# marwie/mageslam

Measured on AMD Instinct MI355X. Metric: frames/sec ORB extract+match @720p; local-BA iters/sec (50 KF, 5k pts), higher is better.
Workload: dtype u8

## Files before the change

### mageslam_amd/csrc/localmap.hip

```cpp
#include <hip/hip_runtime.h>

#include <algorithm>
#include <climits>
#include <cstring>

#include "band_index.hpp"
#include "common.hpp"
#include "lds_sort.hpp"
#include "ordered_take.hpp"

namespace mage {
namespace {

constexpr int LM_MAXT = 4096;
constexpr int LM_CAP = 8;
constexpr int LM_GROUP = 16;
static_assert(LM_MAXT <= OT_MAX_TARGETS, "keypoint indices must fit resolve_in_order's packings");

struct LmRec {
    int n;
    int lo, hi;
    int pad;
    uint32_t e[LM_CAP];
};

__global__ __launch_bounds__(SORT_THREADS) void lm_keys_kernel(LocalMapArgs a, unsigned long long* __restrict__ gkeys)
{
    __shared__ unsigned long long keys[LM_MAXT];
    const int n = (int)*a.nt, tid = threadIdx.x;
    if (*a.nq == 0) return;
    if (n > LM_MAXT) {
        if (tid == 0) atomicOr(a.status, 1u);
        return;
    }
    int P = 1;
    while (P < n) P <<= 1;
    for (int i = tid; i < max(P, SORT_THREADS); i += SORT_THREADS)
        keys[i] = i < n ? ~band_key(a.tkp[i].octave, a.tkp[i].y, (unsigned)i) : 0ull;
    __syncthreads();
    sort_desc(keys, P);
    for (int i = tid; i < n; i += SORT_THREADS) gkeys[i] = ~keys[i];
}

template <typename F>
__device__ __forceinline__ void scan_band(const LocalMapArgs& a, const unsigned long long* keys, int q, int lo, int hi,
                                          int first, int step, F visit)
{
    const float r = a.radius, px = a.qpos[2 * q], py = a.qpos[2 * q + 1];
    const float x0 = px - r, x1 = px + r, y0 = py - r, y1 = py + r;
    const int hide = a.qhide ? a.qhide[q] : -1;
    const uint8_t* qd = a.qdesc + 32ll * q;
    for (int i = lo + first; i < hi; i += step) {
        const int t = (int)(keys[i] & 0xFFFFFFu);
        const float tx = a.tkp[t].x, ty = a.tkp[t].y;
        if (!(tx >= x0 && tx <= x1 && ty >= y0 && ty <= y1) || t == hide) continue;
        const uint32_t d = hamming256(qd, a.tdesc + 32ll * t);
        if ((int)d <= a.max_dist) visit(t, (int)d);
    }
}

__global__ __launch_bounds__(1024) void lm_cand_kernel(LocalMapArgs a, const unsigned long long* __restrict__ keys,
                                                       LmRec* __restrict__ recs)
{
    const int nq = (int)*a.nq, nt = (int)*a.nt;
    if (nt > LM_MAXT || nq > (int)a.q_cap) return;
    const int q = (int)((blockIdx.x * 1024 + threadIdx.x) / LM_GROUP), sub = threadIdx.x % LM_GROUP;
    const bool live = q < nq;
    int lo = 0, hi = 0;
    if (live) {
        const float py = a.qpos[2 * q + 1], r = a.radius;
        const int oq = a.qoct[q];
        lo = lower_bound_keys(keys, nt, band_key(oq, py - r, 0u));
        hi = lower_bound_keys(keys, nt, band_key(oq, py + r, 0xFFFFFFu) + 1ull);
    }
    int n = 0;
    for (int i0 = lo; __any(live && i0 < hi); i0 += LM_GROUP) {
        bool f = false;
        uint32_t ent = 0;
        if (live && i0 + sub < hi) {
            const int i = i0 + sub;
            const int t = (int)(keys[i] & 0xFFFFFFu);
            if (mask_bit(a.mask_words, t))
                scan_band(a, keys, q, i, i + 1, 0, 1, [&](int tt, int d) {
                    f = true;
                    ent = kept_entry(tt, d);
                });
        }
        const int pos = group_append<LM_GROUP>(f, sub, n);
        if (f && pos < LM_CAP) recs[q].e[pos] = ent;
    }
    if (live && sub == 0) {
        recs[q].n = n;
        recs[q].lo = lo;
        recs[q].hi = hi;
    }
}

__global__ __launch_bounds__(1024) void lm_resolve_kernel(LocalMapArgs a, const unsigned long long* __restrict__ keys,
                                                          const LmRec* __restrict__ recs)
{
    __shared__ uint32_t m[LM_MAXT / 32];
    __shared__ int taker[LM_MAXT];
    __shared__ int list[1024];
    __shared__ uint32_t ent[64][LM_CAP];
    __shared__ uint32_t wsum[16];
    const int tid = threadIdx.x, lane = tid & 63, wave = tid >> 6;
    const int nq = (int)*a.nq, nt = (int)*a.nt;
    if (nt > LM_MAXT || nq > (int)a.q_cap) {
        if (tid == 0) atomicOr(a.status, 2u);
        return;
    }
    for (int i = tid; i < LM_MAXT / 32; i += 1024) m[i] = i < (nt + 31) / 32 ? a.mask_words[i] : 0u;
    for (int i = tid; i < LM_MAXT; i += 1024) taker[i] = OT_NO_TAKER;
    __syncthreads();
    for (int b0 = 0; b0 < nq; b0 += 1024) {
        const int q = b0 + tid;
        const bool has = q < nq && recs[q].n > 0;
        if (q < nq) a.result[q] = -1;
        const uint64_t bal = __ballot(has);
        if (lane == 0) wsum[wave] = (uint32_t)__popcll(bal);
        __syncthreads();
        int off = 0, cnt = 0;
        for (int w = 0; w < 16; w++) {
            off += w < wave ? (int)wsum[w] : 0;
            cnt += (int)wsum[w];
        }
        if (has) list[off + __popcll(bal & ((1ull << lane) - 1ull))] = q;
        __syncthreads();
        if (tid < 64)
            resolve_in_order(
                cnt, a.max_dist, a.min_diff, m, taker,
                [&](int k, bool act) {
                    const int qq = act ? list[k] : 0;
                    int n = 0, lo = 0, hi = 0;
                    if (act) {
                        n = recs[qq].n;
                        lo = recs[qq].lo;
                        hi = recs[qq].hi;
                        for (int e = 0; e < LM_CAP && e < n; e++) ent[tid][e] = recs[qq].e[e];
                    }
                    return [=, &a](auto fn) {
                        if (!act) return;
                        if (n <= LM_CAP) {
                            for (int e = 0; e < n; e++) {
                                const uint32_t v = ent[tid][e];
                                if (mask_bit(m, kept_target(v))) fn(kept_target(v), kept_dist(v));
                            }
                        } else {
                            scan_band(a, keys, qq, lo, hi, 0, 1, [&](int t, int d) {
                                if (mask_bit(m, t)) fn(t, d);
                            });
                        }
                    };
                },
                [&](int k, bool ok, int t) {
                    if (ok) a.result[list[k]] = t;
                });
        __syncthreads();
    }
    for (int i = tid; i < (nt + 31) / 32; i += 1024) a.mask_words[i] = m[i];
}

}

size_t local_map_scratch_bytes(uint32_t q_cap)
{
    return ((size_t)LM_MAXT * 8 + 255) / 256 * 256 + (size_t)std::max(q_cap, 1u) * sizeof(LmRec);
}

mage_status local_map_match_launch(const LocalMapArgs& a, void* scratch, hipStream_t st)
{
    unsigned long long* keys = static_cast<unsigned long long*>(scratch);
    LmRec* recs = reinterpret_cast<LmRec*>(static_cast<char*>(scratch) + ((size_t)LM_MAXT * 8 + 255) / 256 * 256);
    if (a.keys)
        keys = const_cast<unsigned long long*>(a.keys);
    else
        launch("localmap.keys", lm_keys_kernel, dim3(1), dim3(SORT_THREADS), 0, st, a, keys);
    const unsigned groups = (unsigned)(((size_t)std::max(a.q_cap, 1u) * LM_GROUP + 1023) / 1024);
    launch("localmap.cand", lm_cand_kernel, dim3(groups), dim3(1024), 0, st, a, (const unsigned long long*)keys, recs);
    launch("localmap.resolve", lm_resolve_kernel, dim3(1), dim3(1024), 0, st, a, (const unsigned long long*)keys,
           (const LmRec*)recs);
    MAGE_HIP(hipGetLastError());
    return MAGE_OK;
}

}

extern "C" mage_status mage_local_map_match(const float* query_pos, const int32_t* query_octave, const uint8_t* query_desc,
                                            const int32_t* query_hide, uint32_t n_query, const mage_keypoint* target_kp,
                                            const uint8_t* target_desc, uint32_t n_target, uint8_t* mask, float radius,
                                            int32_t max_distance, int32_t min_difference, int32_t* result, int device)
{
    using namespace mage;
    MAGE_REQUIRE(mask && (n_target == 0 || (target_kp && target_desc)) &&
                     (n_query == 0 || (query_pos && query_octave && query_desc && result)),
                 MAGE_EINVAL, "null argument");
    MAGE_REQUIRE(n_target <= (uint32_t)LM_MAXT, MAGE_EUNSUPPORTED, "more than 4096 target keypoints");
    MAGE_REQUIRE(max_distance >= -1 && max_distance <= 256, MAGE_EINVAL, "maxHammingDist must be in [-1, 256]");
    if (n_query == 0) return MAGE_OK;
    mage_status r = bind_device(device);
    if (r != MAGE_OK) return r;
    HostScratch* sp = host_scratch(device, SCRATCH_LOCALMAP);
    if (!sp) return MAGE_EDEVICE;
    HostScratch& S = *sp;
    auto al = [](size_t v) { return (v + 255) & ~(size_t)255; };
    const size_t oqp = 0, oqo = al(oqp + 8ull * n_query), oqh = al(oqo + 4ull * n_query), oqd = al(oqh + 4ull * n_query),
                 otk = al(oqd + 32ull * n_query), otd = al(otk + 28ull * std::max(n_target, 1u)),
                 ocnt = al(otd + 32ull * std::max(n_target, 1u)), omw = al(ocnt + 8), ores = al(omw + 4 * (LM_MAXT / 32)),
                 ost = al(ores + 4ull * n_query), oscr = al(ost + 4), total = oscr + local_map_scratch_bytes(n_query);
    if ((r = S.buf.reserve(total)) != MAGE_OK || (r = S.host.reserve(oscr)) != MAGE_OK) return r;
    char* b = S.buf.as<char>();
    char* h = S.host.as<char>();
    std::memcpy(h + oqp, query_pos, 8ull * n_query);
    std::memcpy(h + oqo, query_octave, 4ull * n_query);
    if (query_hide) std::memcpy(h + oqh, query_hide, 4ull * n_query);
    else std::memset(h + oqh, 0xFF, 4ull * n_query);
    std::memcpy(h + oqd, query_desc, 32ull * n_query);
    if (n_target) {
        std::memcpy(h + otk, target_kp, 28ull * n_target);
        std::memcpy(h + otd, target_desc, 32ull * n_target);
    }
    const uint32_t counts[2] = {n_query, n_target};
    std::memcpy(h + ocnt, counts, 8);
    uint32_t* mw = reinterpret_cast<uint32_t*>(h + omw);
    std::memset(mw, 0, 4 * (LM_MAXT / 32));
    for (uint32_t t = 0; t < n_target; t++)
        if (mask[t]) mw[t >> 5] |= 1u << (t & 31);
    std::memset(h + ost, 0, 4);
    MAGE_HIP(hipMemcpyAsync(b, h, oscr, hipMemcpyHostToDevice, S.st));
    LocalMapArgs a{};
    a.qpos = reinterpret_cast<const float*>(b + oqp);
    a.qoct = reinterpret_cast<const int*>(b + oqo);
    a.qhide = reinterpret_cast<const int*>(b + oqh);
    a.qdesc = reinterpret_cast<const uint8_t*>(b + oqd);
    a.nq = reinterpret_cast<const uint32_t*>(b + ocnt);
    a.q_cap = n_query;
    a.tkp = reinterpret_cast<const mage_keypoint*>(b + otk);
    a.tdesc = reinterpret_cast<const uint8_t*>(b + otd);
    a.nt = reinterpret_cast<const uint32_t*>(b + ocnt) + 1;
    a.mask_words = reinterpret_cast<uint32_t*>(b + omw);
    a.radius = radius;
    a.max_dist = max_distance;
    a.min_diff = min_difference;
    a.result = reinterpret_cast<int*>(b + ores);
    a.status = reinterpret_cast<uint32_t*>(b + ost);
    if ((r = local_map_match_launch(a, b + oscr, S.st)) != MAGE_OK) return r;
    MAGE_HIP(hipMemcpyAsync(h + omw, b + omw, oscr - omw, hipMemcpyDeviceToHost, S.st));
    MAGE_HIP(hipStreamSynchronize(S.st));
    MAGE_REQUIRE(*reinterpret_cast<const uint32_t*>(h + ost) == 0, MAGE_EDEVICE, "local map match: bad counts");
    std::memcpy(result, h + ores, 4ull * n_query);
    for (uint32_t t = 0; t < n_target; t++) mask[t] = (mw[t >> 5] >> (t & 31)) & 1u;
    return MAGE_OK;
}
```

### mageslam_amd/csrc/radius.hip

```cpp
#include <hip/hip_runtime.h>

#include <algorithm>
#include <climits>
#include <cstring>

#include "common.hpp"
#include "band_index.hpp"
#include "lds_sort.hpp"

namespace mage {
namespace {

constexpr int RM_MAXT = 4096;
constexpr int RM_STAGE = 2048;

struct RadiusParams {
    const mage_keypoint* qkp;
    const float* qpos;
    const uint8_t* qmask;
    const uint8_t* qdesc;
    const uint32_t* nq;
    long long q_pitch;
    const mage_keypoint* tkp;
    const uint8_t* tmask;
    const uint8_t* tdesc;
    const uint32_t* nt;
    long long t_pitch;
    float radius;
    int max_dist, min_diff;
    unsigned cap;
    int* res;
    mage_dmatch* out;
    uint32_t* n_out;
    uint32_t* status;
    const unsigned long long* bkeys;
    const float2* bxy;
    const uint4* bdesc;
    RadiusFollow follow;
};

__device__ __forceinline__ void radius_done(const RadiusParams& p, int pr, uint32_t n)
{
    p.n_out[pr] = n;
    const RadiusFollow& g = p.follow;
    if (!g.exec) return;
    const uint32_t ns = *g.ns;
    const bool weak = radius_pass_weak(n, ns, g.min_matches, g.ratio);
    const uint32_t run = g.exec[g.k] && weak;
    g.exec[g.k + 1] = run;
    *g.nq_next = run ? ns : 0u;
}

constexpr int RM_GROUP = 16;
constexpr int RM_GROUPS = SORT_THREADS / RM_GROUP;

__device__ __forceinline__ unsigned group_min(unsigned v)
{
#pragma unroll
    for (int off = RM_GROUP / 2; off > 0; off >>= 1) v = min(v, (unsigned)__shfl_xor((int)v, off));
    return v;
}

__device__ void radius_post(const RadiusParams& p, int pr, const int* res, int nq, int ntr, int* bestD, int* cnt,
                            int* wsum, int& s_base)
{
    const int tid = threadIdx.x, lane = tid & 63;
    const int wave = __builtin_amdgcn_readfirstlane(tid >> 6);
    for (int i = tid; i < ntr; i += SORT_THREADS) {
        bestD[i] = INT_MAX;
        cnt[i] = 0;
    }
    __syncthreads();
    for (int q = tid; q < nq; q += SORT_THREADS) {
        const int v = res[q];
        if (v >= 0) atomicMin(&bestD[v >> 9], v & 0x1FF);
    }
    __syncthreads();
    for (int q = tid; q < nq; q += SORT_THREADS) {
        const int v = res[q];
        if (v >= 0 && (v & 0x1FF) == bestD[v >> 9]) atomicAdd(&cnt[v >> 9], 1);
    }
    if (tid == 0) s_base = 0;
    __syncthreads();
    for (int q0 = 0; q0 < nq; q0 += SORT_THREADS) {
        const int q = q0 + tid;
        const int v = q < nq ? res[q] : -1;
        const bool keep = v >= 0 && (v & 0x1FF) == bestD[v >> 9] && cnt[v >> 9] == 1;
        const unsigned long long b = __ballot(keep);
        const int before = __popcll(b & ((1ull << lane) - 1ull));
        if (lane == 0) wsum[wave] = __popcll(b);
        __syncthreads();
        int off = s_base;
        for (int w = 0; w < wave; w++) off += wsum[w];
        if (keep) {
            const int pos = off + before;
            if (pos < (int)p.cap) {
                mage_dmatch m;
                m.query_idx = q;
                m.train_idx = v >> 9;
                m.img_idx = 0;
                m.distance = (float)(v & 0x1FF);
                p.out[(long long)pr * p.cap + pos] = m;
            }
        }
        __syncthreads();
        if (tid == 0) {
            int tot = 0;
            for (int w = 0; w < SORT_THREADS / kWave; w++) tot += wsum[w];
            s_base += tot;
        }
        __syncthreads();
    }
    if (tid == 0) radius_done(p, pr, (uint32_t)s_base);
}

template <bool FUSED>
__global__ __launch_bounds__(SORT_THREADS) void radius_match_kernel(RadiusParams p)
{
    __shared__ unsigned long long keys[RM_MAXT];
    __shared__ float2 sxy[RM_STAGE];
    __shared__ uint4 sdesc[2 * RM_STAGE];
    __shared__ int wsum[SORT_THREADS / kWave];
    __shared__ int s_base;
    const int pr = blockIdx.x, tid = threadIdx.x;
    const int nq = (int)p.nq[pr], ntr = (int)p.nt[pr];
    const mage_keypoint* qkp = p.qkp + pr * p.q_pitch;
    const mage_keypoint* tkp = p.tkp + pr * p.t_pitch;
    const uint8_t* qdesc = p.qdesc + pr * p.q_pitch * 32;
    const uint8_t* tdesc = p.tdesc + pr * p.t_pitch * 32;
    const uint8_t* qmask = p.qmask ? p.qmask + pr * p.q_pitch : nullptr;
    const uint8_t* tmask = p.tmask ? p.tmask + pr * p.t_pitch : nullptr;
    const float* qpos = p.qpos ? p.qpos + 2 * pr * p.q_pitch : nullptr;
    int* res = p.res + pr * p.q_pitch;
    if (nq == 0) {
        if (FUSED && tid == 0) radius_done(p, pr, 0);
        return;
    }
    if (ntr > RM_MAXT || ntr > p.t_pitch || nq > p.q_pitch) {
        if (tid == 0 && blockIdx.y == 0) {
            radius_done(p, pr, 0);
            atomicOr(p.status, ntr > RM_MAXT ? 1u : 2u);
        }
        return;
    }
    const bool staged = ntr <= RM_STAGE;
    if (p.bkeys) {
        const long long tb = pr * p.t_pitch;
        for (int i = tid; i < ntr; i += SORT_THREADS) keys[i] = p.bkeys[tb + i];
        if (staged)
            for (int i = tid; i < 2 * ntr; i += SORT_THREADS) {
                sdesc[i] = p.bdesc[2 * tb + i];
                if (!(i & 1)) sxy[i >> 1] = p.bxy[tb + (i >> 1)];
            }
        __syncthreads();
    } else {
    int P = 1;
    while (P < ntr) P <<= 1;
    for (int i = tid; i < max(P, SORT_THREADS); i += SORT_THREADS)
        keys[i] = i < ntr ? ~band_key(tkp[i].octave, tkp[i].y, (unsigned)i) : 0ull;
    __syncthreads();
    sort_desc(keys, P);
    for (int i = tid; i < ntr; i += SORT_THREADS) keys[i] = ~keys[i];
    __syncthreads();
    if (staged) {
        for (int i = tid; i < 2 * ntr; i += SORT_THREADS) {
            const int t = (int)(keys[i >> 1] & 0xFFFFFFu);
            sdesc[i] = reinterpret_cast<const uint4*>(tdesc + 32 * (long long)t)[i & 1];
            if (!(i & 1)) {
                const bool off = tmask && !tmask[t];
                sxy[i >> 1] = off ? make_float2(__int_as_float(0x7FC00000), 0.f) : make_float2(tkp[t].x, tkp[t].y);
            }
        }
        __syncthreads();
    }
    }

    const float r = p.radius;
    const int group = tid / RM_GROUP, sub = tid % RM_GROUP;
    for (int q = (int)blockIdx.y * RM_GROUPS + group; q < nq; q += RM_GROUPS * (int)gridDim.y) {
        if (qmask && !qmask[q]) {
            if (sub == 0) res[q] = -1;
            continue;
        }
        const float px = qpos ? qpos[2 * q] : qkp[q].x, py = qpos ? qpos[2 * q + 1] : qkp[q].y;
        const int oq = qkp[q].octave;
        const float x0 = px - r, x1 = px + r, y0 = py - r, y1 = py + r;
        const int lo = lower_bound_keys(keys, ntr, band_key(oq, y0, 0u));
        const int hi = lower_bound_keys(keys, ntr, band_key(oq, y1, 0xFFFFFFu) + 1ull);
        uint4 qa = *reinterpret_cast<const uint4*>(qdesc + 32 * (long long)q);
        uint4 qb = *reinterpret_cast<const uint4*>(qdesc + 32 * (long long)q + 16);
        unsigned bestk = 0xFFFFFFFFu;
        for (int i = lo + sub; i < hi; i += RM_GROUP) {
            const int t = (int)(keys[i] & 0xFFFFFFu);
            uint4 ta, tb;
            if (staged) {
                const float2 xy = sxy[i];
                if (!(xy.x >= x0 && xy.x <= x1 && xy.y >= y0 && xy.y <= y1)) continue;
                ta = sdesc[2 * i];
                tb = sdesc[2 * i + 1];
            } else {
                const float tx = tkp[t].x, ty = tkp[t].y;
                if (!(tx >= x0 && tx <= x1 && ty >= y0 && ty <= y1)) continue;
                if (tmask && !tmask[t]) continue;
                ta = *reinterpret_cast<const uint4*>(tdesc + 32 * (long long)t);
                tb = *reinterpret_cast<const uint4*>(tdesc + 32 * (long long)t + 16);
            }
            const unsigned d = __popc(qa.x ^ ta.x) + __popc(qa.y ^ ta.y) + __popc(qa.z ^ ta.z) + __popc(qa.w ^ ta.w) +
                               __popc(qb.x ^ tb.x) + __popc(qb.y ^ tb.y) + __popc(qb.z ^ tb.z) + __popc(qb.w ^ tb.w);
            bestk = min(bestk, d << 12 | (unsigned)t);
        }
        bestk = group_min(bestk);
        const int best = bestk == 0xFFFFFFFFu ? INT_MAX : (int)(bestk >> 12), tbest = (int)(bestk & 0xFFFu);
        if (best > p.max_dist) {
            if (sub == 0) res[q] = -1;
            continue;
        }
        unsigned sec = (unsigned)(p.max_dist + 1);
        for (int i = lo + sub; i < hi; i += RM_GROUP) {
            const int t = (int)(keys[i] & 0xFFFFFFu);
            if (t >= tbest) continue;
            uint4 ta, tb;
            if (staged) {
                const float2 xy = sxy[i];
                if (!(xy.x >= x0 && xy.x <= x1 && xy.y >= y0 && xy.y <= y1)) continue;
                ta = sdesc[2 * i];
                tb = sdesc[2 * i + 1];
            } else {
                const float tx = tkp[t].x, ty = tkp[t].y;
                if (!(tx >= x0 && tx <= x1 && ty >= y0 && ty <= y1)) continue;
                if (tmask && !tmask[t]) continue;
                ta = *reinterpret_cast<const uint4*>(tdesc + 32 * (long long)t);
                tb = *reinterpret_cast<const uint4*>(tdesc + 32 * (long long)t + 16);
            }
            const unsigned d = __popc(qa.x ^ ta.x) + __popc(qa.y ^ ta.y) + __popc(qa.z ^ ta.z) + __popc(qa.w ^ ta.w) +
                               __popc(qb.x ^ tb.x) + __popc(qb.y ^ tb.y) + __popc(qb.z ^ tb.z) + __popc(qb.w ^ tb.w);
            sec = min(sec, d);
        }
        sec = group_min(sec);
        if (sub == 0) res[q] = ((int)sec - best > p.min_diff) ? (tbest << 9 | best) : -1;
    }
    if constexpr (FUSED) {
        __syncthreads();
        int* bestD = reinterpret_cast<int*>(keys);
        radius_post(p, pr, res, nq, ntr, bestD, bestD + RM_MAXT, wsum, s_base);
    }
}

__global__ __launch_bounds__(SORT_THREADS) void radius_post_kernel(RadiusParams p)
{
    __shared__ int bestD[RM_MAXT];
    __shared__ int cnt[RM_MAXT];
    __shared__ int wsum[SORT_THREADS / kWave];
    __shared__ int s_base;
    const int pr = blockIdx.x;
    const int nq = (int)p.nq[pr], ntr = (int)p.nt[pr];
    if (nq == 0) {
        if (threadIdx.x == 0) radius_done(p, pr, 0);
        return;
    }
    if (ntr > RM_MAXT || ntr > p.t_pitch || nq > p.q_pitch) return;
    radius_post(p, pr, p.res + pr * p.q_pitch, nq, ntr, bestD, cnt, wsum, s_base);
}

__global__ __launch_bounds__(SORT_THREADS) void radius_band_index_kernel(const mage_keypoint* __restrict__ tkp,
                                                                         const uint8_t* __restrict__ tdesc,
                                                                         const uint32_t* __restrict__ nt, long long t_pitch,
                                                                         unsigned long long* __restrict__ bkeys,
                                                                         float2* __restrict__ bxy, uint4* __restrict__ bdesc)
{
    __shared__ unsigned long long keys[RM_MAXT];
    const int set = blockIdx.x, tid = threadIdx.x;
    const int ntr = (int)nt[set];
    if (ntr > RM_MAXT || ntr > t_pitch) return;
    const long long tb = set * t_pitch;
    const mage_keypoint* k = tkp + tb;
    int P = 1;
    while (P < ntr) P <<= 1;
    for (int i = tid; i < max(P, SORT_THREADS); i += SORT_THREADS)
        keys[i] = i < ntr ? ~band_key(k[i].octave, k[i].y, (unsigned)i) : 0ull;
    __syncthreads();
    sort_desc(keys, P);
    for (int i = tid; i < ntr; i += SORT_THREADS) {
        const unsigned long long key = ~keys[i];
        const int t = (int)(key & 0xFFFFFFu);
        bkeys[tb + i] = key;
        bxy[tb + i] = make_float2(k[t].x, k[t].y);
        const uint4* d = reinterpret_cast<const uint4*>(tdesc + 32 * (tb + t));
        bdesc[2 * (tb + i)] = d[0];
        bdesc[2 * (tb + i) + 1] = d[1];
    }
}

}

mage_status radius_band_index_launch(const mage_keypoint* d_target_kp, const uint8_t* d_target_desc,
                                     const uint32_t* d_n_target, int64_t target_pitch, uint32_t sets,
                                     unsigned long long* d_keys, float* d_xy, uint32_t* d_desc, hipStream_t st)
{
    if (sets == 0) return MAGE_OK;
    launch("match.radius_index", radius_band_index_kernel, dim3(sets), dim3(SORT_THREADS), 0, st, d_target_kp,
           d_target_desc, d_n_target, (long long)target_pitch, d_keys, reinterpret_cast<float2*>(d_xy),
           reinterpret_cast<uint4*>(d_desc));
    MAGE_HIP(hipGetLastError());
    return MAGE_OK;
}

mage_status radius_match_launch(const RadiusParams& p, uint32_t pairs, hipStream_t st)
{
    const uint32_t split = pairs >= 128 ? 1u : std::min(64u, (256u + pairs - 1) / pairs);
    if (split == 1) {
        launch("match.radius", radius_match_kernel<true>, dim3(pairs), dim3(SORT_THREADS), 0, st, p);
    } else {
        launch("match.radius", radius_match_kernel<false>, dim3(pairs, split), dim3(SORT_THREADS), 0, st, p);
        MAGE_HIP(hipGetLastError());
        launch("match.radius_post", radius_post_kernel, dim3(pairs), dim3(SORT_THREADS), 0, st, p);
    }
    MAGE_HIP(hipGetLastError());
    return MAGE_OK;
}

}

extern "C" {

mage_status mage_radius_match(const mage_keypoint* query_kp, const float* query_pos, const uint8_t* query_mask,
                              const uint8_t* query_desc, uint32_t n_query, const mage_keypoint* target_kp,
                              const uint8_t* target_mask, const uint8_t* target_desc, uint32_t n_target,
                              float radius, int32_t max_distance, int32_t min_difference, mage_dmatch* out,
                              uint32_t cap, uint32_t* n)
{
    using namespace mage;
    MAGE_REQUIRE(n && (cap == 0 || out), MAGE_EINVAL, "null output");
    *n = 0;
    MAGE_REQUIRE((n_query == 0 || (query_kp && query_desc)) && (n_target == 0 || (target_kp && target_desc)),
                 MAGE_EINVAL, "null input");
    MAGE_REQUIRE(n_target <= (uint32_t)RM_MAXT, MAGE_EUNSUPPORTED, "more than 4096 target keypoints");
    MAGE_REQUIRE(max_distance >= -1 && max_distance <= 256, MAGE_EINVAL, "maxHammingDist must be in [-1, 256]");
    if (n_query == 0 || n_target == 0) return MAGE_OK;
    int dev = 0;
    MAGE_HIP(hipGetDevice(&dev));
    mage_status r = bind_device(dev);
    if (r != MAGE_OK) return r;
    HostScratch* sp = host_scratch(dev, SCRATCH_RADIUS);
    if (!sp) return MAGE_EDEVICE;
    HostScratch& S = *sp;
    auto al = [](size_t v) { return (v + 255) & ~(size_t)255; };
    const size_t oqk = 0, otk = al(oqk + 28ull * n_query), oqd = al(otk + 28ull * n_target),
                 otd = al(oqd + 32ull * n_query), oqp = al(otd + 32ull * n_target), oqm = al(oqp + 8ull * n_query),
                 otm = al(oqm + n_query), ocnt = al(otm + n_target), ores = al(ocnt + 16),
                 oout = al(ores + 4ull * n_query), total = oout + 16ull * n_query;
    if ((r = S.buf.reserve(total)) != MAGE_OK || (r = S.host.reserve(total)) != MAGE_OK) return r;
    char* b = S.buf.as<char>();
    char* h = S.host.as<char>();
    std::memcpy(h + oqk, query_kp, 28ull * n_query);
    std::memcpy(h + otk, target_kp, 28ull * n_target);
    std::memcpy(h + oqd, query_desc, 32ull * n_query);
    std::memcpy(h + otd, target_desc, 32ull * n_target);
    if (query_pos) std::memcpy(h + oqp, query_pos, 8ull * n_query);
    if (query_mask) std::memcpy(h + oqm, query_mask, n_query);
    if (target_mask) std::memcpy(h + otm, target_mask, n_target);
    const uint32_t counts[4] = {n_query, n_target, 0, 0};
    std::memcpy(h + ocnt, counts, 16);
    MAGE_HIP(hipMemcpyAsync(b, h, ores, hipMemcpyHostToDevice, S.st));
    RadiusParams p{};
    p.qkp = reinterpret_cast<const mage_keypoint*>(b + oqk);
    p.qpos = query_pos ? reinterpret_cast<const float*>(b + oqp) : nullptr;
    p.qmask = query_mask ? reinterpret_cast<const uint8_t*>(b + oqm) : nullptr;
    p.qdesc = reinterpret_cast<const uint8_t*>(b + oqd);
    p.nq = reinterpret_cast<const uint32_t*>(b + ocnt);
    p.q_pitch = n_query;
    p.tkp = reinterpret_cast<const mage_keypoint*>(b + otk);
    p.tmask = target_mask ? reinterpret_cast<const uint8_t*>(b + otm) : nullptr;
    p.tdesc = reinterpret_cast<const uint8_t*>(b + otd);
    p.nt = reinterpret_cast<const uint32_t*>(b + ocnt) + 1;
    p.t_pitch = n_target;
    p.radius = radius;
    p.max_dist = max_distance;
    p.min_diff = min_difference;
    p.cap = n_query;
    p.res = reinterpret_cast<int*>(b + ores);
    p.out = reinterpret_cast<mage_dmatch*>(b + oout);
    p.n_out = reinterpret_cast<uint32_t*>(b + ocnt) + 2;
    p.status = reinterpret_cast<uint32_t*>(b + ocnt) + 3;
    if ((r = radius_match_launch(p, 1, S.st)) != MAGE_OK) return r;
    MAGE_HIP(hipMemcpyAsync(h + ocnt, b + ocnt, total - ocnt, hipMemcpyDeviceToHost, S.st));
    MAGE_HIP(hipStreamSynchronize(S.st));
    const uint32_t m = reinterpret_cast<const uint32_t*>(h + ocnt)[2];
    if (m > 0 && cap > 0) std::memcpy(out, h + oout, 16ull * (m < cap ? m : cap));
    *n = m < cap ? m : cap;
    MAGE_REQUIRE(m <= cap, MAGE_ECAPACITY, "output capacity too small");
    return MAGE_OK;
}

mage_status mage_radius_match_batch_device(const mage_keypoint* d_query_kp, const float* d_query_pos,
                                           const uint8_t* d_query_desc, int64_t query_pitch,
                                           const uint32_t* d_n_query, const mage_keypoint* d_target_kp,
                                           const uint8_t* d_target_desc, int64_t target_pitch,
                                           const uint32_t* d_n_target, uint32_t pairs, float radius,
                                           int32_t max_distance, int32_t min_difference, int32_t* d_scratch,
                                           mage_dmatch* d_out, uint32_t cap, uint32_t* d_n, uint32_t* d_status,
                                           mage_stream stream)
{
    using namespace mage;
    if (pairs == 0) return MAGE_OK;
    MAGE_REQUIRE(d_query_kp && d_query_desc && d_n_query && d_target_kp && d_target_desc && d_n_target &&
                     d_scratch && d_out && d_n && d_status,
                 MAGE_EINVAL, "null buffer");
    MAGE_REQUIRE(query_pitch > 0 && target_pitch > 0, MAGE_EINVAL, "pitches must be positive");
    MAGE_REQUIRE(max_distance >= -1 && max_distance <= 256, MAGE_EINVAL, "maxHammingDist must be in [-1, 256]");
    RadiusParams p{};
    p.qkp = d_query_kp;
    p.qpos = d_query_pos;
    p.qdesc = d_query_desc;
    p.nq = d_n_query;
    p.q_pitch = query_pitch;
    p.tkp = d_target_kp;
    p.tdesc = d_target_desc;
    p.nt = d_n_target;
    p.t_pitch = target_pitch;
    p.radius = radius;
    p.max_dist = max_distance;
    p.min_diff = min_difference;
    p.cap = cap;
    p.res = d_scratch;
    p.out = d_out;
    p.n_out = d_n;
    p.status = d_status;
    return radius_match_launch(p, pairs, (hipStream_t)stream);
}

}

namespace mage {
mage_status radius_match_indexed(const mage_keypoint* d_query_kp, const float* d_query_pos, const uint8_t* d_query_desc,
                                 int64_t query_pitch, const uint32_t* d_n_query, const mage_keypoint* d_target_kp,
                                 const uint8_t* d_target_desc, int64_t target_pitch, const uint32_t* d_n_target,
                                 const unsigned long long* d_keys, const float* d_xy, const uint32_t* d_desc,
                                 uint32_t pairs, float radius, int32_t max_distance, int32_t min_difference,
                                 int32_t* d_scratch, mage_dmatch* d_out, uint32_t cap, uint32_t* d_n, uint32_t* d_status,
                                 hipStream_t st, const RadiusFollow* follow)
{
    if (pairs == 0) return MAGE_OK;
    MAGE_REQUIRE(!follow || pairs == 1, MAGE_EINVAL, "a RadiusFollow decision is per single pair");
    MAGE_REQUIRE(max_distance >= -1 && max_distance <= 256, MAGE_EINVAL, "maxHammingDist must be in [-1, 256]");
    RadiusParams p{};
    p.qkp = d_query_kp;
    p.qpos = d_query_pos;
    p.qdesc = d_query_desc;
    p.nq = d_n_query;
    p.q_pitch = query_pitch;
    p.tkp = d_target_kp;
    p.tdesc = d_target_desc;
    p.nt = d_n_target;
    p.t_pitch = target_pitch;
    p.radius = radius;
    p.max_dist = max_distance;
    p.min_diff = min_difference;
    p.cap = cap;
    p.res = d_scratch;
    p.out = d_out;
    p.n_out = d_n;
    p.status = d_status;
    p.bkeys = d_keys;
    p.bxy = reinterpret_cast<const float2*>(d_xy);
    p.bdesc = reinterpret_cast<const uint4*>(d_desc);
    if (follow) p.follow = *follow;
    return radius_match_launch(p, pairs, st);
}
}
```

### mageslam_amd/csrc/track.hip

```cpp
#include <hip/hip_runtime.h>

#include <algorithm>
#include <atomic>
#include <chrono>
#include <vector>

#include "common.hpp"
#include "ordered_take.hpp"
#include "track_window.hpp"

namespace mage {
namespace {

using namespace track;

constexpr int TT = 1024;

__device__ void make_keyframe(const TrackBufs& b, const TrackConst& c, uint32_t slot, const mage_keypoint* fk,
                              const uint8_t* fd, uint32_t nf, const Pose& P, uint32_t fid)
{
    float R32[9], t32[3], Cf[3];
    pose_f32(P.R, P.t, R32, t32);
    world_position(R32, t32, Cf);
    const size_t o = (size_t)slot * c.cap;
    if (threadIdx.x < 12) b.kf_pose[12 * slot + threadIdx.x] = threadIdx.x < 9 ? P.R[threadIdx.x] : P.t[threadIdx.x - 9];
    for (uint32_t i = threadIdx.x; i < nf; i += TT) {
        b.kf_ref[o + i] = 0;
        b.kf_own[o + i] = 1;
        b.kf_kp[o + i] = fk[i];
        const uint4* s = reinterpret_cast<const uint4*>(fd + 32ull * i);
        uint4* d = reinterpret_cast<uint4*>(b.kf_desc + 32ull * (o + i));
        d[0] = s[0];
        d[1] = s[1];
        float Pp[3], mvd[3], dmin, dmax;
        backproject_to_plane(fk[i].x, fk[i].y, P, c.K, c.plane_z, fid, i, c.s.map_point_depth_noise, Pp);
        for (int j = 0; j < 3; j++) b.kf_pts[3 * (o + i) + j] = Pp[j];
        point_attributes(Pp, Cf, fk[i].octave, c.fmin, c.fmax, mvd, dmin, dmax);
        for (int j = 0; j < 3; j++) b.kf_mvd[3 * (o + i) + j] = mvd[j];
        b.kf_dmin[o + i] = dmin;
        b.kf_dmax[o + i] = dmax;
    }
}

__device__ __forceinline__ uint32_t ref_slot(const Ctl* ctl, const TrackConst& c)
{
    return (ctl->kf_first + ctl->kf_count - 1) % c.nk;
}

__device__ uint32_t frame_count(const TrackConst& c, const uint32_t* nf, uint32_t* status)
{
    const uint32_t n = *nf;
    if (n > c.cap) {
        if (threadIdx.x == 0) atomicOr(status, 2u);
        return c.cap;
    }
    return n;
}

__global__ __launch_bounds__(TT) void trk_init(TrackBufs b, TrackConst c, const mage_keypoint* fk, const uint8_t* fd,
                                               const uint32_t* nf, double* poses, uint32_t* matches,
                                               uint32_t* inliers, uint8_t* keyframe, uint32_t* status)
{
    const uint32_t n = frame_count(c, nf, status);
    make_keyframe(b, c, 0, fk, fd, n, load_pose(poses), 0u);
    if (threadIdx.x == 0) {
        b.ctl->kf_first = 0;
        b.ctl->kf_count = 1;
        b.ctl->kf_n[0] = n;
        b.ctl->kf_id[0] = 0;
        b.ctl->kf_an[0] = 0;
        b.ctl->halt = 0;
        matches[0] = inliers[0] = n;
        keyframe[0] = 1;
        b.intr4[0] = c.cx;
        b.intr4[1] = c.cy;
        b.intr4[2] = c.fx;
        b.intr4[3] = c.fy;
    }
}

__device__ void project_frame(const TrackBufs& b, const TrackConst& c, int f, const double* poses)
{
    __shared__ float R32[9], t32[3];
    __shared__ uint32_t wsum[TT / 64];
    if (b.ctl->halt) {
        if (threadIdx.x == 0) {
            b.ctl->ns = 0;
            for (int k = 0; k < 3; k++) b.ctl->exec[k] = b.nq[k] = 0;
        }
        return;
    }
    if (threadIdx.x == 0) {
        const Pose p1 = load_pose(poses + 12ll * (f - 1));
        const Pose pred = f < 2 ? p1 : predict(p1, load_pose(poses + 12ll * (f - 2)));
        store_pose(b.pred, pred);
        pose_f32(pred.R, pred.t, R32, t32);
    }
    __syncthreads();
    const uint32_t slot = ref_slot(b.ctl, c), nk = b.ctl->kf_n[slot];
    const size_t o = (size_t)slot * c.cap;
    uint32_t base = 0;
    for (uint32_t c0 = 0; c0 < nk; c0 += TT) {
        const uint32_t i = c0 + threadIdx.x;
        bool front = false;
        float u = 0.f, v = 0.f;
        if (i < nk) {
            const float X[3] = {b.kf_pts[3 * (o + i)], b.kf_pts[3 * (o + i) + 1], b.kf_pts[3 * (o + i) + 2]};
            front = project_front(R32, t32, c.fx, c.fy, c.cx, c.cy, X, u, v);
        }
        uint32_t tot;
        const uint32_t pos = base + block_prefix<TT / 64>(front, wsum, &tot);
        if (front) {
            b.qkp[pos] = b.kf_kp[o + i];
            const uint4* s = reinterpret_cast<const uint4*>(b.kf_desc + 32ull * (o + i));
            uint4* d = reinterpret_cast<uint4*>(b.qdesc + 32ull * pos);
            d[0] = s[0];
            d[1] = s[1];
            b.qpos[2 * pos] = u;
            b.qpos[2 * pos + 1] = v;
            b.sel[pos] = i;
        }
        base += tot;
    }
    if (threadIdx.x == 0) {
        b.ctl->ns = base;
        b.ctl->exec[0] = 1;
        b.ctl->exec[1] = b.ctl->exec[2] = 0;
        b.nq[0] = base;
        b.nq[1] = b.nq[2] = 0;
    }
}

__global__ __launch_bounds__(TT) void trk_gather(TrackBufs b, TrackConst c, const mage_keypoint* fk, int f,
                                                 uint32_t* matches)
{
    if (b.ctl->halt) {
        if (threadIdx.x == 0) {
            b.ctl->lost = 1;
            b.os1[0] = b.os1[1] = 0;
        }
        return;
    }
    const int fin = b.ctl->exec[2] ? 2 : (b.ctl->exec[1] ? 1 : 0);
    const uint32_t n = b.mn[fin];
    const bool lost = n < c.s.min_matches;
    const mage_dmatch* m = b.m + (size_t)fin * c.cap;
    if (!lost) {
        const uint32_t slot = ref_slot(b.ctl, c);
        const size_t o = (size_t)slot * c.cap;
        const int kid = (int)b.ctl->kf_id[slot];
        for (uint32_t k = threadIdx.x; k < n; k += TT) {
            const uint32_t q = b.sel[m[k].query_idx], t = (uint32_t)m[k].train_idx;
            for (int j = 0; j < 3; j++) b.pts1[3 * k + j] = b.kf_pts[3 * (o + q) + j];
            b.uv1[2 * k] = fk[t].x;
            b.uv1[2 * k + 1] = fk[t].y;
            b.info1[k] = refinement_confidence(b.kf_ref[o + q]);
            b.src1[k] = make_int2(kid, (int)q);
        }
    }
    if (threadIdx.x == 0) {
        matches[f] = n;
        b.ctl->lost = lost;
        b.os1[0] = 0;
        b.os1[1] = lost ? 0u : n;
        to_bundler(b.pred, b.pred + 9, b.pos3, b.r9);
    }
}

__device__ void filter_frame(const TrackBufs& b, const TrackConst& c, const uint32_t* nf_ptr)
{
    __shared__ uint32_t wsum[TT / 64];
    const uint32_t n = b.os1[1];
    uint32_t base = 0;
    for (uint32_t c0 = 0; c0 < n; c0 += TT) {
        const uint32_t k = c0 + threadIdx.x;
        const bool keep = k < n && !b.out1[k];
        uint32_t tot;
        const uint32_t pos = base + block_prefix<TT / 64>(keep, wsum, &tot);
        if (keep) {
            for (int j = 0; j < 3; j++) b.pts2[3 * pos + j] = b.pts1[3 * k + j];
            b.uv2[2 * pos] = b.uv1[2 * k];
            b.uv2[2 * pos + 1] = b.uv1[2 * k + 1];
            b.info2[pos] = b.info1[k];
            b.src2[pos] = b.src1[k];
        }
        base += tot;
    }
    if (threadIdx.x == 0) {
        b.os2[0] = 0;
        b.os2[1] = base;
    }
    if (c.s.local_map_keyframes == 0 || b.ctl->lost) return;
    __shared__ uint32_t smask[4096 / 32];
    const uint32_t nf = min(min(*nf_ptr, c.cap), 4096u);
    const uint32_t nk = b.ctl->kf_n[ref_slot(b.ctl, c)];
    for (uint32_t w = threadIdx.x; w < (nf + 31) / 32; w += TT)
        smask[w] = (32 * w + 32 <= nf) ? 0xFFFFFFFFu : ((1u << (nf - 32 * w)) - 1u);
    for (uint32_t i = threadIdx.x; i < nk; i += TT) {
        b.lm_visited[i] = 0;
        b.lm_hide[i] = -1;
    }
    __syncthreads();
    const int fin = b.ctl->exec[2] ? 2 : (b.ctl->exec[1] ? 1 : 0);
    const mage_dmatch* m = b.m + (size_t)fin * c.cap;
    for (uint32_t k = threadIdx.x; k < n; k += TT) {
        const uint32_t q = b.sel[m[k].query_idx], t = (uint32_t)m[k].train_idx;
        if (!b.out1[k]) {
            if (t < nf) atomicAnd(&smask[t >> 5], ~(1u << (t & 31)));
            b.lm_visited[q] = 1;
        } else {
            b.lm_hide[q] = (int32_t)t;
        }
    }
    __syncthreads();
    for (uint32_t w = threadIdx.x; w < (nf + 31) / 32; w += TT) b.lm_mask[w] = smask[w];
}

__device__ void lm_project_frame(const TrackBufs& b, const TrackConst& c)
{
    __shared__ uint32_t wsum[TT / 64];
    const bool off = c.s.local_map_keyframes == 0 || b.ctl->lost;
    if (off || b.os2[1] == 0) {
        if (threadIdx.x == 0) {
            if (!off) b.ctl->lost = 1;
            b.ctl->lm_nq = 0;
        }
        return;
    }
    float R[9], t[3], C[3];
    from_bundler(b.pos3_o1, b.r9_o1, R, t);
    world_position(R, t, C);
    const uint32_t first = b.ctl->kf_first, count = b.ctl->kf_count;
    uint32_t base = 0;
    for (uint32_t si = 0; si < count; si++) {
        const uint32_t slot = (first + si) % c.nk, n = b.ctl->kf_n[slot];
        const bool is_ref = si + 1 == count;
        const size_t o = (size_t)slot * c.cap;
        for (uint32_t c0 = 0; c0 < n; c0 += TT) {
            const uint32_t i = c0 + threadIdx.x;
            bool ok = i < n && !(is_ref && b.lm_visited[i]);
            float px = 0.f, py = 0.f;
            int oc = 0;
            if (ok)
                ok = local_map_candidate(R, t, C, c.fx, c.fy, c.cx, c.cy, c.s, c.log2s, b.kf_pts + 3 * (o + i),
                                         b.kf_mvd + 3 * (o + i), b.kf_dmin[o + i], b.kf_dmax[o + i], px, py, oc);
            uint32_t tot;
            const uint32_t pos = base + block_prefix<TT / 64>(ok, wsum, &tot);
            if (ok && pos < c.qcap) {
                b.lm_qpos[2 * pos] = px;
                b.lm_qpos[2 * pos + 1] = py;
                b.lm_qoct[pos] = oc;
                b.lm_qhide[pos] = is_ref ? b.lm_hide[i] : -1;
                const uint4* sd = reinterpret_cast<const uint4*>(b.kf_desc + 32ull * (o + i));
                uint4* dd = reinterpret_cast<uint4*>(b.lm_qdesc + 32ull * pos);
                dd[0] = sd[0];
                dd[1] = sd[1];
                for (int j = 0; j < 3; j++) b.lm_qpt[3 * pos + j] = b.kf_pts[3 * (o + i) + j];
                b.lm_qsrc[pos] = make_int2((int)b.ctl->kf_id[slot], (int)i);
                b.lm_qinfo[pos] = refinement_confidence(b.kf_ref[o + i]);
            }
            base += tot;
        }
    }
    if (threadIdx.x == 0) b.ctl->lm_nq = min(base, c.qcap);
}

__global__ __launch_bounds__(TT) void trk_lm_assemble(TrackBufs b, const mage_keypoint* fk)
{
    __shared__ uint32_t wsum[TT / 64];
    const uint32_t nq = b.ctl->lm_nq;
    if (b.ctl->lost || nq == 0) return;
    const uint32_t base0 = b.os2[1];
    uint32_t base = base0;
    for (uint32_t c0 = 0; c0 < nq; c0 += TT) {
        const uint32_t q = c0 + threadIdx.x;
        const int r = q < nq ? b.lm_res[q] : -1;
        uint32_t tot;
        const uint32_t pos = base + block_prefix<TT / 64>(r >= 0, wsum, &tot);
        if (r >= 0) {
            for (int j = 0; j < 3; j++) b.pts2[3 * pos + j] = b.lm_qpt[3 * q + j];
            b.uv2[2 * pos] = fk[r].x;
            b.uv2[2 * pos + 1] = fk[r].y;
            b.info2[pos] = b.lm_qinfo[q];
            b.src2[pos] = b.lm_qsrc[q];
        }
        base += tot;
    }
    if (threadIdx.x == 0) b.os2[1] = base;
}

__device__ void finish_frame(const TrackBufs& b, const TrackConst& c, int f, const mage_keypoint* fk,
                             const uint8_t* fd, const uint32_t* nf, double* poses, uint32_t* inliers,
                             uint8_t* keyframe, uint32_t* status)
{
    __shared__ uint32_t wsum[TT / 64];
    __shared__ int s_kf;
    __shared__ uint32_t s_slot;
    __shared__ double sP[12];
    if (b.ctl->halt) return;
    bool lost = b.ctl->lost != 0;
    uint32_t n_in = 0;
    if (!lost) {
        const uint32_t n2 = b.os2[1];
        for (uint32_t c0 = 0; c0 < n2; c0 += TT) {
            const uint32_t k = c0 + threadIdx.x;
            uint32_t tot;
            (void)block_prefix<TT / 64>(k < n2 && !b.out2[k], wsum, &tot);
            n_in += tot;
        }
        if (c.s.local_map_keyframes > 0 && n_in < c.s.min_tracked) lost = true;
    }
    if (threadIdx.x == 0) {
        Pose P;
        from_bundler(b.pos3_o2, b.r9_o2, P.R, P.t);
        if (lost) P = load_pose(b.pred);
        store_pose(poses + 12ll * f, P);
        store_pose(sP, P);
        inliers[f] = lost ? 0u : n_in;
        const uint32_t nk = b.ctl->kf_n[ref_slot(b.ctl, c)];
        s_kf = !lost && (double)n_in < c.s.keyframe_ratio * (double)nk + (double)c.s.keyframe_min;
        keyframe[f] = (uint8_t)s_kf;
        if (s_kf) {
            if (b.ctl->kf_count < c.nk) {
                s_slot = (b.ctl->kf_first + b.ctl->kf_count) % c.nk;
                b.ctl->kf_count++;
            } else {
                s_slot = b.ctl->kf_first;
                b.ctl->kf_first = (b.ctl->kf_first + 1) % c.nk;
            }
        }
    }
    __syncthreads();
    if (s_kf) {
        const uint32_t n = frame_count(c, nf, status);
        make_keyframe(b, c, s_slot, fk, fd, n, load_pose(sP), f);
        const uint32_t n2 = b.os2[1];
        int4* as = b.kf_assoc + (size_t)s_slot * c.acap;
        uint8_t* aa = b.kf_aalive + (size_t)s_slot * c.acap;
        uint32_t base = 0;
        for (uint32_t c0 = 0; c0 < n2; c0 += TT) {
            const uint32_t k = c0 + threadIdx.x;
            const bool in = k < n2 && !b.out2[k];
            uint32_t tot;
            const uint32_t pos = base + block_prefix<TT / 64>(in, wsum, &tot);
            if (in && pos < c.acap) {
                as[pos] = make_int4(b.src2[k].x, b.src2[k].y, __float_as_int(b.uv2[2 * k]), __float_as_int(b.uv2[2 * k + 1]));
                aa[pos] = 1;
            }
            base += tot;
        }
        if (threadIdx.x == 0) {
            b.ctl->kf_n[s_slot] = n;
            b.ctl->kf_id[s_slot] = (uint32_t)f;
            b.ctl->kf_an[s_slot] = min(base, c.acap);
            if (c.s.local_ba && b.ctl->kf_count >= 2) b.ctl->halt = 1;
        }
    }
    if (b.prog && threadIdx.x == 0) {
        if (s_kf && c.s.local_ba && b.ctl->kf_count >= 2) *reinterpret_cast<volatile uint32_t*>(b.prog + 1) = (uint32_t)f;
        __threadfence_system();
        *reinterpret_cast<volatile uint32_t*>(b.prog) = (uint32_t)f;
    }
}

__global__ __launch_bounds__(TT) void trk_project(TrackBufs b, TrackConst c, int f, const double* poses)
{
    project_frame(b, c, f, poses);
}

__global__ __launch_bounds__(TT) void trk_filter(TrackBufs b, TrackConst c, const uint32_t* nf_ptr)
{
    filter_frame(b, c, nf_ptr);
}

__global__ __launch_bounds__(TT) void trk_filter_lm(TrackBufs b, TrackConst c, const uint32_t* nf_ptr)
{
    filter_frame(b, c, nf_ptr);
    __syncthreads();
    lm_project_frame(b, c);
}

__global__ __launch_bounds__(TT) void trk_finish_project(TrackBufs b, TrackConst c, int f, const mage_keypoint* fk,
                                                         const uint8_t* fd, const uint32_t* nf, double* poses,
                                                         uint32_t* inliers, uint8_t* keyframe, uint32_t* status,
                                                         int project_next)
{
    finish_frame(b, c, f, fk, fd, nf, poses, inliers, keyframe, status);
    if (!project_next) return;
    __syncthreads();
    project_frame(b, c, f + 1, poses);
}

}
}

namespace mage {
namespace {

struct PhaseClock {
    bool on = false;
    std::chrono::steady_clock::time_point t;
    char line[512];
    int len = 0;
    void start()
    {
        if (!on) return;
        t = std::chrono::steady_clock::now();
        len = 0;
    }
    void mark(const char* name)
    {
        if (!on) return;
        const auto n = std::chrono::steady_clock::now();
        len += snprintf(line + len, sizeof(line) - len, " %s %.3f", name,
                        std::chrono::duration<double, std::milli>(n - t).count());
        t = n;
    }
    void flush()
    {
        if (on) fprintf(stderr, "local BA window ms:%s\n", line);
    }
};

template <class T>
struct Pinned {
    T* p = nullptr;
    size_t n = 0;
    Pinned() = default;
    Pinned(const Pinned&) = delete;
    Pinned& operator=(const Pinned&) = delete;
    ~Pinned()
    {
        if (p) (void)hipHostFree(p);
    }
    bool resize(size_t m)
    {
        if (m <= n) return true;
        if (p) (void)hipHostFree(p);
        p = nullptr;
        n = 0;
        if (hipHostMalloc(reinterpret_cast<void**>(&p), std::max<size_t>(m, 1) * sizeof(T), hipHostMallocDefault) != hipSuccess)
            return false;
        n = m;
        return true;
    }
    T* data() { return p; }
};

struct BundlerHandle {
    mage_ba* ba = nullptr;
    ~BundlerHandle()
    {
        if (ba) mage_ba_destroy(ba);
    }
};

struct BaSolution {
    std::vector<uint32_t> outl;
    uint32_t nout = 0;
    std::vector<float> pos, r9, xyz;
};

mage_status solve_window(const BaWindow& w, const TrackConst& c, LocalBA& L, int device, BundlerHandle& H, BaSolution& o,
                         PhaseClock& prof)
{
    const uint32_t nr = w.nr, P = (uint32_t)w.keys.size(), E = (uint32_t)w.kept.size();
    const std::vector<float> hw(std::max(w.steps, 1u), w.huber);
    mage_status st;
    if ((st = mage_ba_create(0, device, &H.ba)) != MAGE_OK) return st;
    prof.mark("create");
    if (L.have_lambda && (st = mage_ba_set_lambda(H.ba, L.lambda)) != MAGE_OK) return st;
    if ((st = mage_ba_set_cameras(H.ba, nr, w.pos3.data(), w.r9.data(), w.intr.data(), w.fixed.data())) != MAGE_OK ||
        (st = mage_ba_set_points(H.ba, P, w.xyz.data())) != MAGE_OK ||
        (st = mage_ba_set_observations(H.ba, E, w.uv.data(), w.cam.data(), w.pt.data(), w.info.data())) != MAGE_OK)
        return st;
    prof.mark("setters");
    o.outl.resize(E);
    float ms = 0.f;
    if ((st = mage_ba_step(H.ba, hw.data(), (uint32_t)hw.size(), c.s.ba_max_outlier_error, o.outl.data(), E, &o.nout,
                           &ms)) != MAGE_OK)
        return st;
    prof.mark("step");
    o.pos.resize(3 * nr);
    o.r9.resize(9 * nr);
    o.xyz.resize(3ull * P);
    float lam = 0.f;
    if ((st = mage_ba_get_poses(H.ba, o.pos.data(), o.r9.data())) != MAGE_OK ||
        (st = mage_ba_get_points(H.ba, o.xyz.data())) != MAGE_OK || (st = mage_ba_get_lambda(H.ba, &lam)) != MAGE_OK)
        return st;
    L.have_lambda = true;
    L.lambda = std::max(lam, c.s.min_lambda);
    return MAGE_OK;
}

}
}

extern "C" mage_status mage_track_sequence_device(const mage_keypoint* d_kp, const uint8_t* d_desc, uint32_t pitch,
                                                  const uint32_t* d_n, uint32_t frames, const double K[4],
                                                  const double first_pose[12], double plane_z,
                                                  const mage_track_settings* s, double* poses, uint32_t* matches,
                                                  uint32_t* inliers, uint8_t* keyframe, uint32_t* ba_outliers,
                                                  mage_stream stream)
{
    using namespace mage;
    MAGE_REQUIRE(K && first_pose && s && poses && matches && inliers && keyframe, MAGE_EINVAL, "null argument");
    if (frames == 0) return MAGE_OK;
    MAGE_REQUIRE(d_kp && d_desc && d_n, MAGE_EINVAL, "null features");
    MAGE_REQUIRE(pitch > 0 && pitch <= 4096, MAGE_EINVAL, "frame pitch must be in [1, 4096] keypoints");
    hipStream_t st = (hipStream_t)stream;
    MAGE_REQUIRE(s->local_map_keyframes <= (uint32_t)NKMAX, MAGE_EINVAL, "local_map_keyframes must be <= 8");
    MAGE_REQUIRE(s->refinement_info == refinement_confidence(0), MAGE_EINVAL,
                 "refinement_info must be MapPointRefinementConfidence(0) = 1 - 1/1.5^2");
    const uint32_t NK = std::max(s->local_map_keyframes, 1u);
    const size_t qcap = s->local_map_keyframes > 0 ? (size_t)NK * pitch : 0;
    TrackConst c{};
    c.fx = (float)K[0];
    c.fy = (float)K[1];
    c.cx = (float)K[2];
    c.cy = (float)K[3];
    for (int i = 0; i < 4; i++) c.K[i] = K[i];
    c.plane_z = plane_z;
    c.s = *s;
    c.cap = pitch;
    c.nk = NK;
    c.qcap = (uint32_t)qcap;
    c.acap = (uint32_t)(pitch + qcap);
    octave_factors(s->scale_factor, s->num_levels, c.fmax, c.fmin, &c.log2s);
    const size_t lm_bytes = local_map_scratch_bytes(c.qcap);
    TrackBlock blk{};
    const BlockBinder lay = track_block(blk, c, frames, lm_bytes, nullptr);
    MAGE_REQUIRE(lay.ring_contiguous, MAGE_EINVAL, "track block: the keyframe ring's buffers are not consecutive");
    DeviceBuffer buf;
    mage_status r = buf.reserve(lay.bytes);
    if (r != MAGE_OK) return r;
    char* d = buf.as<char>();
    track_block(blk, c, frames, lm_bytes, d);
    TrackBufs& b = blk.b;
    const float e1 = (float)(s->initial_max_error * s->initial_max_error);
    const float e2 = (float)(s->final_max_error * s->final_max_error);

    auto fail = [&](mage_status st2) {
        (void)hipStreamSynchronize(st);
        buf.release();
        return st2;
    };
    if (hipMemsetAsync(d, 0, lay.bytes, st) != hipSuccess ||
        hipMemcpyAsync(blk.poses, first_pose, 96, hipMemcpyHostToDevice, st) != hipSuccess)
        return fail(MAGE_EDEVICE);
    hipLaunchKernelGGL(trk_init, dim3(1), dim3(TT), 0, st, b, c, d_kp, d_desc, d_n, blk.poses, blk.matches,
                       blk.inliers, blk.keyframe, blk.rstatus);
    const float radius[3] = {s->search_radius, s->wider_search_radius, s->extra_wider_search_radius};
    auto enqueue = [&](uint32_t f, bool project) -> mage_status {
        const mage_keypoint* fk = d_kp + (size_t)f * pitch;
        const uint8_t* fd = d_desc + 32ull * f * pitch;
        const uint32_t* nf = d_n + f;
        const size_t slot = (size_t)(f % BAND_SLOTS);
        mage_status rr;
        if (f == 1 || f % BAND_CHUNK == 0) {
            const uint32_t end = std::min(frames, (f / BAND_CHUNK + 1) * BAND_CHUNK);
            if ((rr = radius_band_index_launch(fk, fd, nf, (int64_t)pitch, end - f, blk.bkeys + slot * pitch,
                                               blk.bxy + 2 * slot * pitch, blk.bdesc + 8 * slot * pitch, st)) !=
                MAGE_OK)
                return rr;
        }
        if (project)
            launch("track.project", trk_project, dim3(1), dim3(TT), 0, st, b, c, (int)f, (const double*)blk.poses);
        for (int k = 0; k < 3; k++) {
            const RadiusFollow follow{&b.ctl->ns, b.ctl->exec, b.nq + k + 1, k, s->min_matches, s->small_match_ratio};
            rr = radius_match_indexed(b.qkp, k < 2 ? b.qpos : nullptr, b.qdesc, (int64_t)pitch, b.nq + k, fk, fd,
                                      (int64_t)pitch, nf, blk.bkeys + slot * pitch, blk.bxy + 2 * slot * pitch,
                                      blk.bdesc + 8 * slot * pitch, 1, radius[k], s->max_hamming,
                                      s->min_hamming_difference, blk.rscratch, b.m + (size_t)k * pitch, pitch,
                                      b.mn + k, blk.rstatus, st, k < 2 ? &follow : nullptr);
            if (rr != MAGE_OK) return rr;
        }
        launch("track.gather", trk_gather, dim3(1), dim3(TT), 0, st, b, c, fk, (int)f, blk.matches);
        rr = mage_ba_pose_batch_device(1, b.pos3, b.r9, b.intr4, b.os1, b.pts1, b.uv1, b.info1, s->initial_steps,
                                       s->initial_huber, e1, b.pos3_o1, b.r9_o1, nullptr, b.out1, b.msq, nullptr,
                                       stream);
        if (rr != MAGE_OK) return rr;
        if (s->local_map_keyframes > 0) {
            launch("track.filter_lm", trk_filter_lm, dim3(1), dim3(TT), 0, st, b, c, nf);
            LocalMapArgs la{};
            la.qpos = b.lm_qpos;
            la.qoct = b.lm_qoct;
            la.qhide = b.lm_qhide;
            la.qdesc = b.lm_qdesc;
            la.nq = &b.ctl->lm_nq;
            la.q_cap = (uint32_t)qcap;
            la.tkp = fk;
            la.tdesc = fd;
            la.nt = nf;
            la.mask_words = b.lm_mask;
            la.radius = s->match_search_radius;
            la.max_dist = s->local_max_hamming;
            la.min_diff = s->local_min_hamming_difference;
            la.result = b.lm_res;
            la.status = b.lm_status;
            la.keys = blk.bkeys + slot * pitch;
            if ((rr = local_map_match_launch(la, b.lm_scratch, st)) != MAGE_OK) return rr;
            launch("track.lm_assemble", trk_lm_assemble, dim3(1), dim3(TT), 0, st, b, fk);
        } else {
            launch("track.filter", trk_filter, dim3(1), dim3(TT), 0, st, b, c, nf);
        }
        rr = mage_ba_pose_batch_device(1, b.pos3_o1, b.r9_o1, b.intr4, b.os2, b.pts2, b.uv2, b.info2, s->final_steps,
                                       s->final_huber, e2, b.pos3_o2, b.r9_o2, nullptr, b.out2, b.msq + 1, nullptr,
                                       stream);
        if (rr != MAGE_OK) return rr;
        launch("track.finish", trk_finish_project, dim3(1), dim3(TT), 0, st, b, c, (int)f, fk, fd, nf, blk.poses,
               blk.inliers, blk.keyframe, blk.rstatus, (int)(f + 1 < frames));
        return MAGE_OK;
    };
    if (ba_outliers)
        for (uint32_t f = 0; f < frames; f++) ba_outliers[f] = 0xFFFFFFFFu;
    if (!s->local_ba) {
        for (uint32_t f = 1; f < frames; f++)
            if ((r = enqueue(f, f == 1)) != MAGE_OK) return fail(r);
    } else {
        int dev = 0;
        if (hipGetDevice(&dev) != hipSuccess) return fail(MAGE_EDEVICE);
        MappedBuffer prog;
        if ((r = prog.reserve(64)) != MAGE_OK) return fail(r);
        volatile uint32_t* hp = prog.host<volatile uint32_t>();
        hp[0] = 0;
        hp[1] = 0;
        b.prog = prog.device<uint32_t>();
        Pinned<uint8_t> mirror;
        Pinned<uint32_t> zero;
        const size_t mbytes = lay.ring_end - lay.ring_begin;
        LocalBA L;
        PhaseClock prof;
        {
            const char* e = getenv("MAGE_TRACK_PROFILE");
            prof.on = e && *e == '1';
        }
        std::vector<uint8_t> changed(NK);
        uint32_t next = 1;
        bool need_project = true;
        constexpr uint32_t DEPTH = 2;
        for (uint32_t f = 1; f < frames; f++) {
            while (next < frames && next <= f + DEPTH) {
                if ((r = enqueue(next, need_project)) != MAGE_OK) return fail(r);
                need_project = false;
                next++;
            }
            const auto t0 = std::chrono::steady_clock::now();
            while (hp[0] < f) {
                if (std::chrono::steady_clock::now() - t0 > std::chrono::milliseconds(50)) {
                    if (hipStreamSynchronize(st) != hipSuccess) return fail(MAGE_EDEVICE);
                    if (hp[0] < f) return fail(MAGE_EDEVICE);
                }
            }
            std::atomic_thread_fence(std::memory_order_acquire);
            if (hp[1] != f) continue;
            prof.start();
            if (hipStreamSynchronize(st) != hipSuccess) return fail(MAGE_EDEVICE);
            prof.mark("drain");
            Ctl hc;
            if (hipMemcpy(&hc, b.ctl, sizeof(Ctl), hipMemcpyDeviceToHost) != hipSuccess) return fail(MAGE_EDEVICE);
            if (!mirror.resize(mbytes) || !zero.resize(1)) return fail(MAGE_ENOMEM);
            *zero.data() = 0;
            if (hipMemcpyAsync(mirror.data(), d + lay.ring_begin, mbytes, hipMemcpyDeviceToHost, st) != hipSuccess ||
                hipStreamSynchronize(st) != hipSuccess)
                return fail(MAGE_EDEVICE);
            HostRing R = host_ring(c, frames, lm_bytes, mirror.data(), hc);
            prof.mark("ring D2H");
            std::fill(changed.begin(), changed.end(), 0);
            const BaWindow w = build_window(R, c, L);
            if (w.valid) {
                prof.mark("window");
                BundlerHandle H;
                BaSolution o;
                if ((r = solve_window(w, c, L, dev, H, o, prof)) != MAGE_OK) return fail(r);
                apply_window(R, c, w, o.outl.data(), o.nout, o.pos.data(), o.r9.data(), o.xyz.data(), changed);
                prof.mark("get + apply");
                if (ba_outliers) ba_outliers[f] = o.nout;
            }
            bool any = false;
            for (uint32_t k = 0; k < NK; k++) any = any || changed[k];
            if (any && hipMemcpyAsync(d + lay.moved_begin, mirror.data() + (lay.moved_begin - lay.ring_begin),
                                      lay.ring_end - lay.moved_begin, hipMemcpyHostToDevice, st) != hipSuccess)
                return fail(MAGE_EDEVICE);
            const uint32_t newest = (hc.kf_first + hc.kf_count - 1) % NK;
            if (hipMemcpyAsync(blk.poses + 12ull * f, &R.v.kf_pose[12 * newest], 96, hipMemcpyHostToDevice, st) !=
                    hipSuccess ||
                hipMemcpyAsync(&b.ctl->halt, zero.data(), 4, hipMemcpyHostToDevice, st) != hipSuccess)
                return fail(MAGE_EDEVICE);
            prof.mark("write-back");
            prof.flush();
            next = f + 1;
            need_project = true;
        }
        if (hipStreamSynchronize(st) != hipSuccess) return fail(MAGE_EDEVICE);
    }
    if (hipGetLastError() != hipSuccess) return fail(MAGE_EDEVICE);
    uint32_t rst = 0, lst = 0;
    if (hipMemcpyAsync(poses, blk.poses, 96ull * frames, hipMemcpyDeviceToHost, st) != hipSuccess ||
        hipMemcpyAsync(matches, blk.matches, 4ull * frames, hipMemcpyDeviceToHost, st) != hipSuccess ||
        hipMemcpyAsync(inliers, blk.inliers, 4ull * frames, hipMemcpyDeviceToHost, st) != hipSuccess ||
        hipMemcpyAsync(keyframe, blk.keyframe, frames, hipMemcpyDeviceToHost, st) != hipSuccess ||
        hipMemcpyAsync(&rst, blk.rstatus, 4, hipMemcpyDeviceToHost, st) != hipSuccess ||
        hipMemcpyAsync(&lst, b.lm_status, 4, hipMemcpyDeviceToHost, st) != hipSuccess ||
        hipStreamSynchronize(st) != hipSuccess)
        return fail(MAGE_EDEVICE);
    buf.release();
    MAGE_REQUIRE(!(rst & 1u), MAGE_ECAPACITY, "a frame has more than 4096 keypoints");
    MAGE_REQUIRE(!(rst & 2u), MAGE_ECAPACITY, "a frame's keypoint count exceeds the frame pitch");
    MAGE_REQUIRE(lst == 0, MAGE_ECAPACITY, "local-map search: a frame has more than 4096 keypoints");
    return MAGE_OK;
}
```

Baseline: 425,400.

## Fuse tracking radius-match passes and local-map resolve into single-workgroup control kernels

The first radius-match pass now runs as a split launch. Its post-processing, the two follow-up radius passes and the gather step are fused into one workgroup kernel (trk_match_tail), replacing several per-pass launches. The local-map resolve is likewise fused with the assemble step into trk_lm_resolve. This aims to cut kernel launch count and inter-kernel gaps in the per-frame tracking chain. In exchange, the later radius passes run in a single workgroup instead of a potentially wider grid, which may lower parallelism when many queries are present.

```diff
diff --git a/mageslam_amd/csrc/localmap.hip b/mageslam_amd/csrc/localmap.hip
--- a/mageslam_amd/csrc/localmap.hip
+++ b/mageslam_amd/csrc/localmap.hip
@@ -7,22 +7,13 @@
 #include "band_index.hpp"
 #include "common.hpp"
 #include "lds_sort.hpp"
+#include "localmap_resolve.hpp"
 #include "ordered_take.hpp"
 
 namespace mage {
 namespace {
 
-constexpr int LM_MAXT = 4096;
-constexpr int LM_CAP = 8;
 constexpr int LM_GROUP = 16;
-static_assert(LM_MAXT <= OT_MAX_TARGETS, "keypoint indices must fit resolve_in_order's packings");
-
-struct LmRec {
-    int n;
-    int lo, hi;
-    int pad;
-    uint32_t e[LM_CAP];
-};
 
 __global__ __launch_bounds__(SORT_THREADS) void lm_keys_kernel(LocalMapArgs a, unsigned long long* __restrict__ gkeys)
 {
@@ -40,23 +31,6 @@
     __syncthreads();
     sort_desc(keys, P);
     for (int i = tid; i < n; i += SORT_THREADS) gkeys[i] = ~keys[i];
-}
-
-template <typename F>
-__device__ __forceinline__ void scan_band(const LocalMapArgs& a, const unsigned long long* keys, int q, int lo, int hi,
-                                          int first, int step, F visit)
-{
-    const float r = a.radius, px = a.qpos[2 * q], py = a.qpos[2 * q + 1];
-    const float x0 = px - r, x1 = px + r, y0 = py - r, y1 = py + r;
-    const int hide = a.qhide ? a.qhide[q] : -1;
-    const uint8_t* qd = a.qdesc + 32ll * q;
-    for (int i = lo + first; i < hi; i += step) {
-        const int t = (int)(keys[i] & 0xFFFFFFu);
-        const float tx = a.tkp[t].x, ty = a.tkp[t].y;
-        if (!(tx >= x0 && tx <= x1 && ty >= y0 && ty <= y1) || t == hide) continue;
-        const uint32_t d = hamming256(qd, a.tdesc + 32ll * t);
-        if ((int)d <= a.max_dist) visit(t, (int)d);
-    }
 }
 
 __global__ __launch_bounds__(1024) void lm_cand_kernel(LocalMapArgs a, const unsigned long long* __restrict__ keys,
@@ -99,66 +73,7 @@
 __global__ __launch_bounds__(1024) void lm_resolve_kernel(LocalMapArgs a, const unsigned long long* __restrict__ keys,
                                                           const LmRec* __restrict__ recs)
 {
-    __shared__ uint32_t m[LM_MAXT / 32];
-    __shared__ int taker[LM_MAXT];
-    __shared__ int list[1024];
-    __shared__ uint32_t ent[64][LM_CAP];
-    __shared__ uint32_t wsum[16];
-    const int tid = threadIdx.x, lane = tid & 63, wave = tid >> 6;
-    const int nq = (int)*a.nq, nt = (int)*a.nt;
-    if (nt > LM_MAXT || nq > (int)a.q_cap) {
-        if (tid == 0) atomicOr(a.status, 2u);
-        return;
-    }
-    for (int i = tid; i < LM_MAXT / 32; i += 1024) m[i] = i < (nt + 31) / 32 ? a.mask_words[i] : 0u;
-    for (int i = tid; i < LM_MAXT; i += 1024) taker[i] = OT_NO_TAKER;
-    __syncthreads();
-    for (int b0 = 0; b0 < nq; b0 += 1024) {
-        const int q = b0 + tid;
-        const bool has = q < nq && recs[q].n > 0;
-        if (q < nq) a.result[q] = -1;
-        const uint64_t bal = __ballot(has);
-        if (lane == 0) wsum[wave] = (uint32_t)__popcll(bal);
-        __syncthreads();
-        int off = 0, cnt = 0;
-        for (int w = 0; w < 16; w++) {
-            off += w < wave ? (int)wsum[w] : 0;
-            cnt += (int)wsum[w];
-        }
-        if (has) list[off + __popcll(bal & ((1ull << lane) - 1ull))] = q;
-        __syncthreads();
-        if (tid < 64)
-            resolve_in_order(
-                cnt, a.max_dist, a.min_diff, m, taker,
-                [&](int k, bool act) {
-                    const int qq = act ? list[k] : 0;
-                    int n = 0, lo = 0, hi = 0;
-                    if (act) {
-                        n = recs[qq].n;
-                        lo = recs[qq].lo;
-                        hi = recs[qq].hi;
-                        for (int e = 0; e < LM_CAP && e < n; e++) ent[tid][e] = recs[qq].e[e];
-                    }
-                    return [=, &a](auto fn) {
-                        if (!act) return;
-                        if (n <= LM_CAP) {
-                            for (int e = 0; e < n; e++) {
-                                const uint32_t v = ent[tid][e];
-                                if (mask_bit(m, kept_target(v))) fn(kept_target(v), kept_dist(v));
-                            }
-                        } else {
-                            scan_band(a, keys, qq, lo, hi, 0, 1, [&](int t, int d) {
-                                if (mask_bit(m, t)) fn(t, d);
-                            });
-                        }
-                    };
-                },
-                [&](int k, bool ok, int t) {
-                    if (ok) a.result[list[k]] = t;
-                });
-        __syncthreads();
-    }
-    for (int i = tid; i < (nt + 31) / 32; i += 1024) a.mask_words[i] = m[i];
+    lm_resolve(a, keys, recs);
 }
 
 }
@@ -168,7 +83,8 @@
     return ((size_t)LM_MAXT * 8 + 255) / 256 * 256 + (size_t)std::max(q_cap, 1u) * sizeof(LmRec);
 }
 
-mage_status local_map_match_launch(const LocalMapArgs& a, void* scratch, hipStream_t st)
+mage_status local_map_cand_launch(const LocalMapArgs& a, void* scratch, hipStream_t st, const unsigned long long** keys_out,
+                                  const LmRec** recs_out)
 {
     unsigned long long* keys = static_cast<unsigned long long*>(scratch);
     LmRec* recs = reinterpret_cast<LmRec*>(static_cast<char*>(scratch) + ((size_t)LM_MAXT * 8 + 255) / 256 * 256);
@@ -178,8 +94,19 @@
         launch("localmap.keys", lm_keys_kernel, dim3(1), dim3(SORT_THREADS), 0, st, a, keys);
     const unsigned groups = (unsigned)(((size_t)std::max(a.q_cap, 1u) * LM_GROUP + 1023) / 1024);
     launch("localmap.cand", lm_cand_kernel, dim3(groups), dim3(1024), 0, st, a, (const unsigned long long*)keys, recs);
-    launch("localmap.resolve", lm_resolve_kernel, dim3(1), dim3(1024), 0, st, a, (const unsigned long long*)keys,
-           (const LmRec*)recs);
+    MAGE_HIP(hipGetLastError());
+    *keys_out = keys;
+    *recs_out = recs;
+    return MAGE_OK;
+}
+
+mage_status local_map_match_launch(const LocalMapArgs& a, void* scratch, hipStream_t st)
+{
+    const unsigned long long* keys = nullptr;
+    const LmRec* recs = nullptr;
+    const mage_status r = local_map_cand_launch(a, scratch, st, &keys, &recs);
+    if (r != MAGE_OK) return r;
+    launch("localmap.resolve", lm_resolve_kernel, dim3(1), dim3(1024), 0, st, a, keys, recs);
     MAGE_HIP(hipGetLastError());
     return MAGE_OK;
 }
diff --git a/mageslam_amd/csrc/localmap_resolve.hpp b/mageslam_amd/csrc/localmap_resolve.hpp
--- /dev/null
+++ b/mageslam_amd/csrc/localmap_resolve.hpp
@@ -0,0 +1,106 @@
+#pragma once
+#include <hip/hip_runtime.h>
+
+#include "band_index.hpp"
+#include "common.hpp"
+#include "ordered_take.hpp"
+
+namespace mage {
+
+constexpr int LM_MAXT = 4096;
+constexpr int LM_CAP = 8;
+static_assert(LM_MAXT <= OT_MAX_TARGETS, "keypoint indices must fit resolve_in_order's packings");
+
+struct LmRec {
+    int n;
+    int lo, hi;
+    int pad;
+    uint32_t e[LM_CAP];
+};
+
+mage_status local_map_cand_launch(const LocalMapArgs& a, void* scratch, hipStream_t st, const unsigned long long** keys,
+                                  const LmRec** recs);
+
+template <typename F>
+__device__ __forceinline__ void scan_band(const LocalMapArgs& a, const unsigned long long* keys, int q, int lo, int hi,
+                                          int first, int step, F visit)
+{
+    const float r = a.radius, px = a.qpos[2 * q], py = a.qpos[2 * q + 1];
+    const float x0 = px - r, x1 = px + r, y0 = py - r, y1 = py + r;
+    const int hide = a.qhide ? a.qhide[q] : -1;
+    const uint8_t* qd = a.qdesc + 32ll * q;
+    for (int i = lo + first; i < hi; i += step) {
+        const int t = (int)(keys[i] & 0xFFFFFFu);
+        const float tx = a.tkp[t].x, ty = a.tkp[t].y;
+        if (!(tx >= x0 && tx <= x1 && ty >= y0 && ty <= y1) || t == hide) continue;
+        const uint32_t d = hamming256(qd, a.tdesc + 32ll * t);
+        if ((int)d <= a.max_dist) visit(t, (int)d);
+    }
+}
+
+__device__ __forceinline__ void lm_resolve(const LocalMapArgs& a, const unsigned long long* __restrict__ keys,
+                                           const LmRec* __restrict__ recs)
+{
+    __shared__ uint32_t m[LM_MAXT / 32];
+    __shared__ int taker[LM_MAXT];
+    __shared__ int list[1024];
+    __shared__ uint32_t ent[64][LM_CAP];
+    __shared__ uint32_t wsum[16];
+    const int tid = threadIdx.x, lane = tid & 63, wave = tid >> 6;
+    const int nq = (int)*a.nq, nt = (int)*a.nt;
+    if (nt > LM_MAXT || nq > (int)a.q_cap) {
+        if (tid == 0) atomicOr(a.status, 2u);
+        return;
+    }
+    for (int i = tid; i < LM_MAXT / 32; i += 1024) m[i] = i < (nt + 31) / 32 ? a.mask_words[i] : 0u;
+    for (int i = tid; i < LM_MAXT; i += 1024) taker[i] = OT_NO_TAKER;
+    __syncthreads();
+    for (int b0 = 0; b0 < nq; b0 += 1024) {
+        const int q = b0 + tid;
+        const bool has = q < nq && recs[q].n > 0;
+        if (q < nq) a.result[q] = -1;
+        const uint64_t bal = __ballot(has);
+        if (lane == 0) wsum[wave] = (uint32_t)__popcll(bal);
+        __syncthreads();
+        int off = 0, cnt = 0;
+        for (int w = 0; w < 16; w++) {
+            off += w < wave ? (int)wsum[w] : 0;
+            cnt += (int)wsum[w];
+        }
+        if (has) list[off + __popcll(bal & ((1ull << lane) - 1ull))] = q;
+        __syncthreads();
+        if (tid < 64)
+            resolve_in_order(
+                cnt, a.max_dist, a.min_diff, m, taker,
+                [&](int k, bool act) {
+                    const int qq = act ? list[k] : 0;
+                    int n = 0, lo = 0, hi = 0;
+                    if (act) {
+                        n = recs[qq].n;
+                        lo = recs[qq].lo;
+                        hi = recs[qq].hi;
+                        for (int e = 0; e < LM_CAP && e < n; e++) ent[tid][e] = recs[qq].e[e];
+                    }
+                    return [=, &a](auto fn) {
+                        if (!act) return;
+                        if (n <= LM_CAP) {
+                            for (int e = 0; e < n; e++) {
+                                const uint32_t v = ent[tid][e];
+                                if (mask_bit(m, kept_target(v))) fn(kept_target(v), kept_dist(v));
+                            }
+                        } else {
+                            scan_band(a, keys, qq, lo, hi, 0, 1, [&](int t, int d) {
+                                if (mask_bit(m, t)) fn(t, d);
+                            });
+                        }
+                    };
+                },
+                [&](int k, bool ok, int t) {
+                    if (ok) a.result[list[k]] = t;
+                });
+        __syncthreads();
+    }
+    for (int i = tid; i < (nt + 31) / 32; i += 1024) a.mask_words[i] = m[i];
+}
+
+}
diff --git a/mageslam_amd/csrc/radius.hip b/mageslam_amd/csrc/radius.hip
--- a/mageslam_amd/csrc/radius.hip
+++ b/mageslam_amd/csrc/radius.hip
@@ -7,112 +7,10 @@
 #include "common.hpp"
 #include "band_index.hpp"
 #include "lds_sort.hpp"
+#include "radius_pair.hpp"
 
 namespace mage {
 namespace {
-
-constexpr int RM_MAXT = 4096;
-constexpr int RM_STAGE = 2048;
-
-struct RadiusParams {
-    const mage_keypoint* qkp;
-    const float* qpos;
-    const uint8_t* qmask;
-    const uint8_t* qdesc;
-    const uint32_t* nq;
-    long long q_pitch;
-    const mage_keypoint* tkp;
-    const uint8_t* tmask;
-    const uint8_t* tdesc;
-    const uint32_t* nt;
-    long long t_pitch;
-    float radius;
-    int max_dist, min_diff;
-    unsigned cap;
-    int* res;
-    mage_dmatch* out;
-    uint32_t* n_out;
-    uint32_t* status;
-    const unsigned long long* bkeys;
-    const float2* bxy;
-    const uint4* bdesc;
-    RadiusFollow follow;
-};
-
-__device__ __forceinline__ void radius_done(const RadiusParams& p, int pr, uint32_t n)
-{
-    p.n_out[pr] = n;
-    const RadiusFollow& g = p.follow;
-    if (!g.exec) return;
-    const uint32_t ns = *g.ns;
-    const bool weak = radius_pass_weak(n, ns, g.min_matches, g.ratio);
-    const uint32_t run = g.exec[g.k] && weak;
-    g.exec[g.k + 1] = run;
-    *g.nq_next = run ? ns : 0u;
-}
-
-constexpr int RM_GROUP = 16;
-constexpr int RM_GROUPS = SORT_THREADS / RM_GROUP;
-
-__device__ __forceinline__ unsigned group_min(unsigned v)
-{
-#pragma unroll
-    for (int off = RM_GROUP / 2; off > 0; off >>= 1) v = min(v, (unsigned)__shfl_xor((int)v, off));
-    return v;
-}
-
-__device__ void radius_post(const RadiusParams& p, int pr, const int* res, int nq, int ntr, int* bestD, int* cnt,
-                            int* wsum, int& s_base)
-{
-    const int tid = threadIdx.x, lane = tid & 63;
-    const int wave = __builtin_amdgcn_readfirstlane(tid >> 6);
-    for (int i = tid; i < ntr; i += SORT_THREADS) {
-        bestD[i] = INT_MAX;
-        cnt[i] = 0;
-    }
-    __syncthreads();
-    for (int q = tid; q < nq; q += SORT_THREADS) {
-        const int v = res[q];
-        if (v >= 0) atomicMin(&bestD[v >> 9], v & 0x1FF);
-    }
-    __syncthreads();
-    for (int q = tid; q < nq; q += SORT_THREADS) {
-        const int v = res[q];
-        if (v >= 0 && (v & 0x1FF) == bestD[v >> 9]) atomicAdd(&cnt[v >> 9], 1);
-    }
-    if (tid == 0) s_base = 0;
-    __syncthreads();
-    for (int q0 = 0; q0 < nq; q0 += SORT_THREADS) {
-        const int q = q0 + tid;
-        const int v = q < nq ? res[q] : -1;
-        const bool keep = v >= 0 && (v & 0x1FF) == bestD[v >> 9] && cnt[v >> 9] == 1;
-        const unsigned long long b = __ballot(keep);
-        const int before = __popcll(b & ((1ull << lane) - 1ull));
-        if (lane == 0) wsum[wave] = __popcll(b);
-        __syncthreads();
-        int off = s_base;
-        for (int w = 0; w < wave; w++) off += wsum[w];
-        if (keep) {
-            const int pos = off + before;
-            if (pos < (int)p.cap) {
-                mage_dmatch m;
-                m.query_idx = q;
-                m.train_idx = v >> 9;
-                m.img_idx = 0;
-                m.distance = (float)(v & 0x1FF);
-                p.out[(long long)pr * p.cap + pos] = m;
-            }
-        }
-        __syncthreads();
-        if (tid == 0) {
-            int tot = 0;
-            for (int w = 0; w < SORT_THREADS / kWave; w++) tot += wsum[w];
-            s_base += tot;
-        }
-        __syncthreads();
-    }
-    if (tid == 0) radius_done(p, pr, (uint32_t)s_base);
-}
 
 template <bool FUSED>
 __global__ __launch_bounds__(SORT_THREADS) void radius_match_kernel(RadiusParams p)
@@ -122,128 +20,9 @@
     __shared__ uint4 sdesc[2 * RM_STAGE];
     __shared__ int wsum[SORT_THREADS / kWave];
     __shared__ int s_base;
-    const int pr = blockIdx.x, tid = threadIdx.x;
-    const int nq = (int)p.nq[pr], ntr = (int)p.nt[pr];
-    const mage_keypoint* qkp = p.qkp + pr * p.q_pitch;
-    const mage_keypoint* tkp = p.tkp + pr * p.t_pitch;
-    const uint8_t* qdesc = p.qdesc + pr * p.q_pitch * 32;
-    const uint8_t* tdesc = p.tdesc + pr * p.t_pitch * 32;
-    const uint8_t* qmask = p.qmask ? p.qmask + pr * p.q_pitch : nullptr;
-    const uint8_t* tmask = p.tmask ? p.tmask + pr * p.t_pitch : nullptr;
-    const float* qpos = p.qpos ? p.qpos + 2 * pr * p.q_pitch : nullptr;
-    int* res = p.res + pr * p.q_pitch;
-    if (nq == 0) {
-        if (FUSED && tid == 0) radius_done(p, pr, 0);
-        return;
-    }
-    if (ntr > RM_MAXT || ntr > p.t_pitch || nq > p.q_pitch) {
-        if (tid == 0 && blockIdx.y == 0) {
-            radius_done(p, pr, 0);
-            atomicOr(p.status, ntr > RM_MAXT ? 1u : 2u);
-        }
-        return;
-    }
-    const bool staged = ntr <= RM_STAGE;
-    if (p.bkeys) {
-        const long long tb = pr * p.t_pitch;
-        for (int i = tid; i < ntr; i += SORT_THREADS) keys[i] = p.bkeys[tb + i];
-        if (staged)
-            for (int i = tid; i < 2 * ntr; i += SORT_THREADS) {
-                sdesc[i] = p.bdesc[2 * tb + i];
-                if (!(i & 1)) sxy[i >> 1] = p.bxy[tb + (i >> 1)];
-            }
-        __syncthreads();
-    } else {
-    int P = 1;
-    while (P < ntr) P <<= 1;
-    for (int i = tid; i < max(P, SORT_THREADS); i += SORT_THREADS)
-        keys[i] = i < ntr ? ~band_key(tkp[i].octave, tkp[i].y, (unsigned)i) : 0ull;
-    __syncthreads();
-    sort_desc(keys, P);
-    for (int i = tid; i < ntr; i += SORT_THREADS) keys[i] = ~keys[i];
-    __syncthreads();
-    if (staged) {
-        for (int i = tid; i < 2 * ntr; i += SORT_THREADS) {
-            const int t = (int)(keys[i >> 1] & 0xFFFFFFu);
-            sdesc[i] = reinterpret_cast<const uint4*>(tdesc + 32 * (long long)t)[i & 1];
-            if (!(i & 1)) {
-                const bool off = tmask && !tmask[t];
-                sxy[i >> 1] = off ? make_float2(__int_as_float(0x7FC00000), 0.f) : make_float2(tkp[t].x, tkp[t].y);
-            }
-        }
-        __syncthreads();
-    }
-    }
-
-    const float r = p.radius;
-    const int group = tid / RM_GROUP, sub = tid % RM_GROUP;
-    for (int q = (int)blockIdx.y * RM_GROUPS + group; q < nq; q += RM_GROUPS * (int)gridDim.y) {
-        if (qmask && !qmask[q]) {
-            if (sub == 0) res[q] = -1;
-            continue;
-        }
-        const float px = qpos ? qpos[2 * q] : qkp[q].x, py = qpos ? qpos[2 * q + 1] : qkp[q].y;
-        const int oq = qkp[q].octave;
-        const float x0 = px - r, x1 = px + r, y0 = py - r, y1 = py + r;
-        const int lo = lower_bound_keys(keys, ntr, band_key(oq, y0, 0u));
-        const int hi = lower_bound_keys(keys, ntr, band_key(oq, y1, 0xFFFFFFu) + 1ull);
-        uint4 qa = *reinterpret_cast<const uint4*>(qdesc + 32 * (long long)q);
-        uint4 qb = *reinterpret_cast<const uint4*>(qdesc + 32 * (long long)q + 16);
-        unsigned bestk = 0xFFFFFFFFu;
-        for (int i = lo + sub; i < hi; i += RM_GROUP) {
-            const int t = (int)(keys[i] & 0xFFFFFFu);
-            uint4 ta, tb;
-            if (staged) {
-                const float2 xy = sxy[i];
-                if (!(xy.x >= x0 && xy.x <= x1 && xy.y >= y0 && xy.y <= y1)) continue;
-                ta = sdesc[2 * i];
-                tb = sdesc[2 * i + 1];
-            } else {
-                const float tx = tkp[t].x, ty = tkp[t].y;
-                if (!(tx >= x0 && tx <= x1 && ty >= y0 && ty <= y1)) continue;
-                if (tmask && !tmask[t]) continue;
-                ta = *reinterpret_cast<const uint4*>(tdesc + 32 * (long long)t);
-                tb = *reinterpret_cast<const uint4*>(tdesc + 32 * (long long)t + 16);
-            }
-            const unsigned d = __popc(qa.x ^ ta.x) + __popc(qa.y ^ ta.y) + __popc(qa.z ^ ta.z) + __popc(qa.w ^ ta.w) +
-                               __popc(qb.x ^ tb.x) + __popc(qb.y ^ tb.y) + __popc(qb.z ^ tb.z) + __popc(qb.w ^ tb.w);
-            bestk = min(bestk, d << 12 | (unsigned)t);
-        }
-        bestk = group_min(bestk);
-        const int best = bestk == 0xFFFFFFFFu ? INT_MAX : (int)(bestk >> 12), tbest = (int)(bestk & 0xFFFu);
-        if (best > p.max_dist) {
-            if (sub == 0) res[q] = -1;
-            continue;
-        }
-        unsigned sec = (unsigned)(p.max_dist + 1);
-        for (int i = lo + sub; i < hi; i += RM_GROUP) {
-            const int t = (int)(keys[i] & 0xFFFFFFu);
-            if (t >= tbest) continue;
-            uint4 ta, tb;
-            if (staged) {
-                const float2 xy = sxy[i];
-                if (!(xy.x >= x0 && xy.x <= x1 && xy.y >= y0 && xy.y <= y1)) continue;
-                ta = sdesc[2 * i];
-                tb = sdesc[2 * i + 1];
-            } else {
-                const float tx = tkp[t].x, ty = tkp[t].y;
-                if (!(tx >= x0 && tx <= x1 && ty >= y0 && ty <= y1)) continue;
-                if (tmask && !tmask[t]) continue;
-                ta = *reinterpret_cast<const uint4*>(tdesc + 32 * (long long)t);
-                tb = *reinterpret_cast<const uint4*>(tdesc + 32 * (long long)t + 16);
-            }
-            const unsigned d = __popc(qa.x ^ ta.x) + __popc(qa.y ^ ta.y) + __popc(qa.z ^ ta.z) + __popc(qa.w ^ ta.w) +
-                               __popc(qb.x ^ tb.x) + __popc(qb.y ^ tb.y) + __popc(qb.z ^ tb.z) + __popc(qb.w ^ tb.w);
-            sec = min(sec, d);
-        }
-        sec = group_min(sec);
-        if (sub == 0) res[q] = ((int)sec - best > p.min_diff) ? (tbest << 9 | best) : -1;
-    }
-    if constexpr (FUSED) {
-        __syncthreads();
-        int* bestD = reinterpret_cast<int*>(keys);
-        radius_post(p, pr, res, nq, ntr, bestD, bestD + RM_MAXT, wsum, s_base);
-    }
+    const int pr = blockIdx.x;
+    radius_match_pair<FUSED>(p, pr, (int)p.nq[pr], (int)blockIdx.y, (int)gridDim.y,
+                             RadiusLds{keys, sxy, sdesc, wsum, &s_base});
 }
 
 __global__ __launch_bounds__(SORT_THREADS) void radius_post_kernel(RadiusParams p)
@@ -253,13 +32,7 @@
     __shared__ int wsum[SORT_THREADS / kWave];
     __shared__ int s_base;
     const int pr = blockIdx.x;
-    const int nq = (int)p.nq[pr], ntr = (int)p.nt[pr];
-    if (nq == 0) {
-        if (threadIdx.x == 0) radius_done(p, pr, 0);
-        return;
-    }
-    if (ntr > RM_MAXT || ntr > p.t_pitch || nq > p.q_pitch) return;
-    radius_post(p, pr, p.res + pr * p.q_pitch, nq, ntr, bestD, cnt, wsum, s_base);
+    radius_post_pair(p, pr, (int)p.nq[pr], bestD, cnt, wsum, s_base);
 }
 
 __global__ __launch_bounds__(SORT_THREADS) void radius_band_index_kernel(const mage_keypoint* __restrict__ tkp,
@@ -301,6 +74,13 @@
     launch("match.radius_index", radius_band_index_kernel, dim3(sets), dim3(SORT_THREADS), 0, st, d_target_kp,
            d_target_desc, d_n_target, (long long)target_pitch, d_keys, reinterpret_cast<float2*>(d_xy),
            reinterpret_cast<uint4*>(d_desc));
+    MAGE_HIP(hipGetLastError());
+    return MAGE_OK;
+}
+
+mage_status radius_match_split_launch(const RadiusParams& p, uint32_t split, hipStream_t st)
+{
+    launch("match.radius", radius_match_kernel<false>, dim3(1, split), dim3(SORT_THREADS), 0, st, p);
     MAGE_HIP(hipGetLastError());
     return MAGE_OK;
 }
diff --git a/mageslam_amd/csrc/radius_pair.hpp b/mageslam_amd/csrc/radius_pair.hpp
--- /dev/null
+++ b/mageslam_amd/csrc/radius_pair.hpp
@@ -0,0 +1,283 @@
+#pragma once
+#include <hip/hip_runtime.h>
+
+#include <climits>
+
+#include "band_index.hpp"
+#include "common.hpp"
+#include "lds_sort.hpp"
+
+namespace mage {
+
+constexpr int RM_MAXT = 4096;
+constexpr int RM_STAGE = 2048;
+
+struct RadiusParams {
+    const mage_keypoint* qkp;
+    const float* qpos;
+    const uint8_t* qmask;
+    const uint8_t* qdesc;
+    const uint32_t* nq;
+    long long q_pitch;
+    const mage_keypoint* tkp;
+    const uint8_t* tmask;
+    const uint8_t* tdesc;
+    const uint32_t* nt;
+    long long t_pitch;
+    float radius;
+    int max_dist, min_diff;
+    unsigned cap;
+    int* res;
+    mage_dmatch* out;
+    uint32_t* n_out;
+    uint32_t* status;
+    const unsigned long long* bkeys;
+    const float2* bxy;
+    const uint4* bdesc;
+    RadiusFollow follow;
+};
+
+mage_status radius_match_split_launch(const RadiusParams& p, uint32_t split, hipStream_t st);
+
+struct RadiusLds {
+    unsigned long long* keys;
+    float2* sxy;
+    uint4* sdesc;
+    int* wsum;
+    int* s_base;
+    uint32_t* next = nullptr;
+};
+static_assert(2 * RM_MAXT * sizeof(int) <= RM_MAXT * sizeof(unsigned long long), "bestD + cnt must fit the keys");
+
+__device__ __forceinline__ uint32_t radius_decide(uint32_t* n_out, const RadiusFollow& g, uint32_t n,
+                                                  uint32_t* next = nullptr)
+{
+    *n_out = n;
+    uint32_t nq_next = 0u;
+    if (g.exec) {
+        const uint32_t ns = *g.ns;
+        const bool weak = radius_pass_weak(n, ns, g.min_matches, g.ratio);
+        const uint32_t run = g.exec[g.k] && weak;
+        g.exec[g.k + 1] = run;
+        nq_next = run ? ns : 0u;
+        *g.nq_next = nq_next;
+    }
+    if (next) *next = nq_next;
+    return nq_next;
+}
+
+__device__ __forceinline__ uint32_t radius_done(const RadiusParams& p, int pr, uint32_t n, uint32_t* next = nullptr)
+{
+    return radius_decide(p.n_out + pr, p.follow, n, next);
+}
+
+constexpr int RM_GROUP = 16;
+constexpr int RM_GROUPS = SORT_THREADS / RM_GROUP;
+
+__device__ __forceinline__ unsigned radius_group_min(unsigned v)
+{
+#pragma unroll
+    for (int off = RM_GROUP / 2; off > 0; off >>= 1) v = min(v, (unsigned)__shfl_xor((int)v, off));
+    return v;
+}
+
+__device__ inline void radius_post(const RadiusParams& p, int pr, const int* res, int nq, int ntr, int* bestD, int* cnt,
+                                   int* wsum, int& s_base, uint32_t* next = nullptr)
+{
+    const int tid = threadIdx.x, lane = tid & 63;
+    const int wave = __builtin_amdgcn_readfirstlane(tid >> 6);
+    for (int i = tid; i < ntr; i += SORT_THREADS) {
+        bestD[i] = INT_MAX;
+        cnt[i] = 0;
+    }
+    __syncthreads();
+    for (int q = tid; q < nq; q += SORT_THREADS) {
+        const int v = res[q];
+        if (v >= 0) atomicMin(&bestD[v >> 9], v & 0x1FF);
+    }
+    __syncthreads();
+    for (int q = tid; q < nq; q += SORT_THREADS) {
+        const int v = res[q];
+        if (v >= 0 && (v & 0x1FF) == bestD[v >> 9]) atomicAdd(&cnt[v >> 9], 1);
+    }
+    if (tid == 0) s_base = 0;
+    __syncthreads();
+    for (int q0 = 0; q0 < nq; q0 += SORT_THREADS) {
+        const int q = q0 + tid;
+        const int v = q < nq ? res[q] : -1;
+        const bool keep = v >= 0 && (v & 0x1FF) == bestD[v >> 9] && cnt[v >> 9] == 1;
+        const unsigned long long b = __ballot(keep);
+        const int before = __popcll(b & ((1ull << lane) - 1ull));
+        if (lane == 0) wsum[wave] = __popcll(b);
+        __syncthreads();
+        int off = s_base;
+        for (int w = 0; w < wave; w++) off += wsum[w];
+        if (keep) {
+            const int pos = off + before;
+            if (pos < (int)p.cap) {
+                mage_dmatch m;
+                m.query_idx = q;
+                m.train_idx = v >> 9;
+                m.img_idx = 0;
+                m.distance = (float)(v & 0x1FF);
+                p.out[(long long)pr * p.cap + pos] = m;
+            }
+        }
+        __syncthreads();
+        if (tid == 0) {
+            int tot = 0;
+            for (int w = 0; w < SORT_THREADS / kWave; w++) tot += wsum[w];
+            s_base += tot;
+        }
+        __syncthreads();
+    }
+    if (tid == 0) radius_done(p, pr, (uint32_t)s_base, next);
+}
+
+__device__ inline void radius_post_pair(const RadiusParams& p, int pr, int nq, int* bestD, int* cnt, int* wsum,
+                                        int& s_base, uint32_t* next = nullptr)
+{
+    const int ntr = (int)p.nt[pr];
+    if (nq == 0) {
+        if (threadIdx.x == 0) radius_done(p, pr, 0, next);
+        return;
+    }
+    if (ntr > RM_MAXT || ntr > p.t_pitch || nq > p.q_pitch) {
+        if (next && threadIdx.x == 0) *next = p.follow.exec ? *p.follow.nq_next : 0u;
+        return;
+    }
+    radius_post(p, pr, p.res + pr * p.q_pitch, nq, ntr, bestD, cnt, wsum, s_base, next);
+}
+
+template <bool FUSED, bool INDEXED = false>
+__device__ inline void radius_match_pair(const RadiusParams& p, int pr, int nq, int y_slot, int y_count,
+                                         const RadiusLds& lds)
+{
+    unsigned long long* keys = lds.keys;
+    float2* sxy = lds.sxy;
+    uint4* sdesc = lds.sdesc;
+    const int tid = threadIdx.x;
+    const int ntr = (int)p.nt[pr];
+    const mage_keypoint* qkp = p.qkp + pr * p.q_pitch;
+    const mage_keypoint* tkp = p.tkp + pr * p.t_pitch;
+    const uint8_t* qdesc = p.qdesc + pr * p.q_pitch * 32;
+    const uint8_t* tdesc = p.tdesc + pr * p.t_pitch * 32;
+    const uint8_t* qmask = p.qmask ? p.qmask + pr * p.q_pitch : nullptr;
+    const uint8_t* tmask = p.tmask ? p.tmask + pr * p.t_pitch : nullptr;
+    const float* qpos = p.qpos ? p.qpos + 2 * pr * p.q_pitch : nullptr;
+    int* res = p.res + pr * p.q_pitch;
+    if (nq == 0) {
+        if (FUSED && tid == 0) radius_done(p, pr, 0, lds.next);
+        return;
+    }
+    if (ntr > RM_MAXT || ntr > p.t_pitch || nq > p.q_pitch) {
+        if (tid == 0 && y_slot == 0) {
+            radius_done(p, pr, 0, lds.next);
+            atomicOr(p.status, ntr > RM_MAXT ? 1u : 2u);
+        }
+        return;
+    }
+    const bool staged = ntr <= RM_STAGE;
+    if (INDEXED || p.bkeys) {
+        const long long tb = pr * p.t_pitch;
+        for (int i = tid; i < ntr; i += SORT_THREADS) keys[i] = p.bkeys[tb + i];
+        if (staged)
+            for (int i = tid; i < 2 * ntr; i += SORT_THREADS) {
+                sdesc[i] = p.bdesc[2 * tb + i];
+                if (!(i & 1)) sxy[i >> 1] = p.bxy[tb + (i >> 1)];
+            }
+        __syncthreads();
+    } else {
+    int P = 1;
+    while (P < ntr) P <<= 1;
+    for (int i = tid; i < max(P, SORT_THREADS); i += SORT_THREADS)
+        keys[i] = i < ntr ? ~band_key(tkp[i].octave, tkp[i].y, (unsigned)i) : 0ull;
+    __syncthreads();
+    sort_desc(keys, P);
+    for (int i = tid; i < ntr; i += SORT_THREADS) keys[i] = ~keys[i];
+    __syncthreads();
+    if (staged) {
+        for (int i = tid; i < 2 * ntr; i += SORT_THREADS) {
+            const int t = (int)(keys[i >> 1] & 0xFFFFFFu);
+            sdesc[i] = reinterpret_cast<const uint4*>(tdesc + 32 * (long long)t)[i & 1];
+            if (!(i & 1)) {
+                const bool off = tmask && !tmask[t];
+                sxy[i >> 1] = off ? make_float2(__int_as_float(0x7FC00000), 0.f) : make_float2(tkp[t].x, tkp[t].y);
+            }
+        }
+        __syncthreads();
+    }
+    }
+
+    const float r = p.radius;
+    const int group = tid / RM_GROUP, sub = tid % RM_GROUP;
+    for (int q = y_slot * RM_GROUPS + group; q < nq; q += RM_GROUPS * y_count) {
+        if (qmask && !qmask[q]) {
+            if (sub == 0) res[q] = -1;
+            continue;
+        }
+        const float px = qpos ? qpos[2 * q] : qkp[q].x, py = qpos ? qpos[2 * q + 1] : qkp[q].y;
+        const int oq = qkp[q].octave;
+        const float x0 = px - r, x1 = px + r, y0 = py - r, y1 = py + r;
+        const int lo = lower_bound_keys(keys, ntr, band_key(oq, y0, 0u));
+        const int hi = lower_bound_keys(keys, ntr, band_key(oq, y1, 0xFFFFFFu) + 1ull);
+        uint4 qa = *reinterpret_cast<const uint4*>(qdesc + 32 * (long long)q);
+        uint4 qb = *reinterpret_cast<const uint4*>(qdesc + 32 * (long long)q + 16);
+        unsigned bestk = 0xFFFFFFFFu;
+        for (int i = lo + sub; i < hi; i += RM_GROUP) {
+            const int t = (int)(keys[i] & 0xFFFFFFu);
+            uint4 ta, tb;
+            if (staged) {
+                const float2 xy = sxy[i];
+                if (!(xy.x >= x0 && xy.x <= x1 && xy.y >= y0 && xy.y <= y1)) continue;
+                ta = sdesc[2 * i];
+                tb = sdesc[2 * i + 1];
+            } else {
+                const float tx = tkp[t].x, ty = tkp[t].y;
+                if (!(tx >= x0 && tx <= x1 && ty >= y0 && ty <= y1)) continue;
+                if (tmask && !tmask[t]) continue;
+                ta = *reinterpret_cast<const uint4*>(tdesc + 32 * (long long)t);
+                tb = *reinterpret_cast<const uint4*>(tdesc + 32 * (long long)t + 16);
+            }
+            const unsigned d = __popc(qa.x ^ ta.x) + __popc(qa.y ^ ta.y) + __popc(qa.z ^ ta.z) + __popc(qa.w ^ ta.w) +
+                               __popc(qb.x ^ tb.x) + __popc(qb.y ^ tb.y) + __popc(qb.z ^ tb.z) + __popc(qb.w ^ tb.w);
+            bestk = min(bestk, d << 12 | (unsigned)t);
+        }
+        bestk = radius_group_min(bestk);
+        const int best = bestk == 0xFFFFFFFFu ? INT_MAX : (int)(bestk >> 12), tbest = (int)(bestk & 0xFFFu);
+        if (best > p.max_dist) {
+            if (sub == 0) res[q] = -1;
+            continue;
+        }
+        unsigned sec = (unsigned)(p.max_dist + 1);
+        for (int i = lo + sub; i < hi; i += RM_GROUP) {
+            const int t = (int)(keys[i] & 0xFFFFFFu);
+            if (t >= tbest) continue;
+            uint4 ta, tb;
+            if (staged) {
+                const float2 xy = sxy[i];
+                if (!(xy.x >= x0 && xy.x <= x1 && xy.y >= y0 && xy.y <= y1)) continue;
+                ta = sdesc[2 * i];
+                tb = sdesc[2 * i + 1];
+            } else {
+                const float tx = tkp[t].x, ty = tkp[t].y;
+                if (!(tx >= x0 && tx <= x1 && ty >= y0 && ty <= y1)) continue;
+                if (tmask && !tmask[t]) continue;
+                ta = *reinterpret_cast<const uint4*>(tdesc + 32 * (long long)t);
+                tb = *reinterpret_cast<const uint4*>(tdesc + 32 * (long long)t + 16);
+            }
+            const unsigned d = __popc(qa.x ^ ta.x) + __popc(qa.y ^ ta.y) + __popc(qa.z ^ ta.z) + __popc(qa.w ^ ta.w) +
+                               __popc(qb.x ^ tb.x) + __popc(qb.y ^ tb.y) + __popc(qb.z ^ tb.z) + __popc(qb.w ^ tb.w);
+            sec = min(sec, d);
+        }
+        sec = radius_group_min(sec);
+        if (sub == 0) res[q] = ((int)sec - best > p.min_diff) ? (tbest << 9 | best) : -1;
+    }
+    if constexpr (FUSED) {
+        __syncthreads();
+        int* bestD = reinterpret_cast<int*>(keys);
+        radius_post(p, pr, res, nq, ntr, bestD, bestD + RM_MAXT, lds.wsum, *lds.s_base, lds.next);
+    }
+}
+
+}
diff --git a/mageslam_amd/csrc/track.hip b/mageslam_amd/csrc/track.hip
--- a/mageslam_amd/csrc/track.hip
+++ b/mageslam_amd/csrc/track.hip
@@ -6,7 +6,9 @@
 #include <vector>
 
 #include "common.hpp"
+#include "localmap_resolve.hpp"
 #include "ordered_take.hpp"
+#include "radius_pair.hpp"
 #include "track_window.hpp"
 
 namespace mage {
@@ -15,6 +17,7 @@
 using namespace track;
 
 constexpr int TT = 1024;
+static_assert(TT == SORT_THREADS, "the control kernels run RadiusMatch pairs in their own workgroup");
 
 __device__ void make_keyframe(const TrackBufs& b, const TrackConst& c, uint32_t slot, const mage_keypoint* fk,
                               const uint8_t* fd, uint32_t nf, const Pose& P, uint32_t fid)
@@ -131,8 +134,8 @@
     }
 }
 
-__global__ __launch_bounds__(TT) void trk_gather(TrackBufs b, TrackConst c, const mage_keypoint* fk, int f,
-                                                 uint32_t* matches)
+__device__ __forceinline__ void gather_frame(const TrackBufs& b, const TrackConst& c, const mage_keypoint* fk, int f,
+                                             uint32_t* matches)
 {
     if (b.ctl->halt) {
         if (threadIdx.x == 0) {
@@ -265,7 +268,7 @@
     if (threadIdx.x == 0) b.ctl->lm_nq = min(base, c.qcap);
 }
 
-__global__ __launch_bounds__(TT) void trk_lm_assemble(TrackBufs b, const mage_keypoint* fk)
+__device__ __forceinline__ void lm_assemble_frame(const TrackBufs& b, const mage_keypoint* fk)
 {
     __shared__ uint32_t wsum[TT / 64];
     const uint32_t nq = b.ctl->lm_nq;
@@ -378,6 +381,56 @@
     filter_frame(b, c, nf_ptr);
     __syncthreads();
     lm_project_frame(b, c);
+}
+
+__global__ __launch_bounds__(TT) void trk_match_tail(RadiusParams p, float radius1, float radius2, TrackBufs b,
+                                                     TrackConst c, const mage_keypoint* fk, int f, uint32_t* matches)
+{
+    __shared__ unsigned long long keys[RM_MAXT];
+    __shared__ float2 sxy[RM_STAGE];
+    __shared__ uint4 sdesc[2 * RM_STAGE];
+    __shared__ int wsum[TT / kWave];
+    __shared__ int s_base;
+    __shared__ uint32_t s_nq[4];
+    int* bestD = reinterpret_cast<int*>(keys);
+    radius_post_pair(p, 0, (int)p.nq[0], bestD, bestD + RM_MAXT, wsum, s_base, &s_nq[1]);
+    for (int k = 1; k < 3; k++) {
+        __syncthreads();
+        const int nqk = (int)s_nq[k];
+        if (nqk == 0) {
+            if (threadIdx.x == 0) {
+                RadiusFollow g = p.follow;
+                g.nq_next = p.follow.nq_next + 1;
+                g.k = 1;
+                if (k == 1) radius_decide(p.n_out + 1, g, 0);
+                g.exec = nullptr;
+                radius_decide(p.n_out + 2, g, 0);
+            }
+            break;
+        }
+        RadiusParams pk = p;
+        pk.radius = k == 1 ? radius1 : radius2;
+        if (k == 2) pk.qpos = nullptr;
+        pk.nq = p.nq + k;
+        pk.out = p.out + (size_t)k * p.cap;
+        pk.n_out = p.n_out + k;
+        pk.follow.k = k;
+        pk.follow.nq_next = p.follow.nq_next + k;
+        if (k == 2) pk.follow.exec = nullptr;
+        const RadiusLds lds{keys, sxy, sdesc, wsum, &s_base, &s_nq[k + 1]};
+        radius_match_pair<true, true>(pk, 0, nqk, 0, 1, lds);
+    }
+    __syncthreads();
+    gather_frame(b, c, fk, f, matches);
+}
+
+__global__ __launch_bounds__(TT) void trk_lm_resolve(LocalMapArgs a, const unsigned long long* __restrict__ keys,
+                                                     const LmRec* __restrict__ recs, TrackBufs b,
+                                                     const mage_keypoint* fk)
+{
+    lm_resolve(a, keys, recs);
+    __syncthreads();
+    lm_assemble_frame(b, fk);
 }
 
 __global__ __launch_bounds__(TT) void trk_finish_project(TrackBufs b, TrackConst c, int f, const mage_keypoint* fk,
@@ -566,16 +619,32 @@
         }
         if (project)
             launch("track.project", trk_project, dim3(1), dim3(TT), 0, st, b, c, (int)f, (const double*)blk.poses);
-        for (int k = 0; k < 3; k++) {
-            const RadiusFollow follow{&b.ctl->ns, b.ctl->exec, b.nq + k + 1, k, s->min_matches, s->small_match_ratio};
-            rr = radius_match_indexed(b.qkp, k < 2 ? b.qpos : nullptr, b.qdesc, (int64_t)pitch, b.nq + k, fk, fd,
-                                      (int64_t)pitch, nf, blk.bkeys + slot * pitch, blk.bxy + 2 * slot * pitch,
-                                      blk.bdesc + 8 * slot * pitch, 1, radius[k], s->max_hamming,
-                                      s->min_hamming_difference, blk.rscratch, b.m + (size_t)k * pitch, pitch,
-                                      b.mn + k, blk.rstatus, st, k < 2 ? &follow : nullptr);
-            if (rr != MAGE_OK) return rr;
-        }
-        launch("track.gather", trk_gather, dim3(1), dim3(TT), 0, st, b, c, fk, (int)f, blk.matches);
+        MAGE_REQUIRE(s->max_hamming >= -1 && s->max_hamming <= 256, MAGE_EINVAL, "maxHammingDist must be in [-1, 256]");
+        RadiusParams p{};
+        p.qkp = b.qkp;
+        p.qpos = b.qpos;
+        p.qdesc = b.qdesc;
+        p.nq = b.nq;
+        p.q_pitch = pitch;
+        p.tkp = fk;
+        p.tdesc = fd;
+        p.nt = nf;
+        p.t_pitch = pitch;
+        p.radius = radius[0];
+        p.max_dist = s->max_hamming;
+        p.min_diff = s->min_hamming_difference;
+        p.cap = pitch;
+        p.res = blk.rscratch;
+        p.out = b.m;
+        p.n_out = b.mn;
+        p.status = blk.rstatus;
+        p.bkeys = blk.bkeys + slot * pitch;
+        p.bxy = reinterpret_cast<const float2*>(blk.bxy + 2 * slot * pitch);
+        p.bdesc = reinterpret_cast<const uint4*>(blk.bdesc + 8 * slot * pitch);
+        p.follow = RadiusFollow{&b.ctl->ns, b.ctl->exec, b.nq + 1, 0, s->min_matches, s->small_match_ratio};
+        if ((rr = radius_match_split_launch(p, 64, st)) != MAGE_OK) return rr;
+        launch("track.match_tail", trk_match_tail, dim3(1), dim3(TT), 0, st, p, radius[1], radius[2], b, c, fk, (int)f,
+               blk.matches);
         rr = mage_ba_pose_batch_device(1, b.pos3, b.r9, b.intr4, b.os1, b.pts1, b.uv1, b.info1, s->initial_steps,
                                        s->initial_huber, e1, b.pos3_o1, b.r9_o1, nullptr, b.out1, b.msq, nullptr,
                                        stream);
@@ -599,8 +668,10 @@
             la.result = b.lm_res;
             la.status = b.lm_status;
             la.keys = blk.bkeys + slot * pitch;
-            if ((rr = local_map_match_launch(la, b.lm_scratch, st)) != MAGE_OK) return rr;
-            launch("track.lm_assemble", trk_lm_assemble, dim3(1), dim3(TT), 0, st, b, fk);
+            const unsigned long long* lkeys = nullptr;
+            const LmRec* lrecs = nullptr;
+            if ((rr = local_map_cand_launch(la, b.lm_scratch, st, &lkeys, &lrecs)) != MAGE_OK) return rr;
+            launch("track.lm_resolve", trk_lm_resolve, dim3(1), dim3(TT), 0, st, la, lkeys, lrecs, b, fk);
         } else {
             launch("track.filter", trk_filter, dim3(1), dim3(TT), 0, st, b, c, nf);
         }
```

Result: no change. 425,200 (-0.0%).
